# xuanvinh1997/llm-fp8

Measured on AMD Instinct MI355X. Metric: train tokens/sec + FP8 GEMM % of MFMA peak, Llama-3.2-3B seq512 b16, higher is better.
Workload: dtype fp8 (E4M3/E5M2 operands, fp32 accumulate, bf16 activations); 1 GPU; llama-3.2-3b (28 layers) full fine-tuning step, batch 16/GPU x seq 512, fp8_scenario=default (te_llama counterpart, lm_head FP8 under the outer recipe), random-init weights, synthetic tokens; route=fused, global_batch=16, seq_len=512, parallelism=single

## Files before the change

### llm_fp8_amd/csrc/mi_gemm.hip

```cpp
#include "mi_gemm_dev.h"
#include <algorithm>
#include <atomic>
#include <cstdlib>
#include <cstring>
#include <type_traits>

namespace mi {

template <int OUT>
__device__ __forceinline__ void store4(void* D, int64_t ldd, int64_t m, int64_t n0, v4f v) {
  if (OUT == 0) {
    uint2 p = make_uint2(pack_bf16x2(v[0], v[1]), pack_bf16x2(v[2], v[3]));
    *reinterpret_cast<uint2*>(reinterpret_cast<uint16_t*>(D) + m * ldd + n0) = p;
  } else {
    *reinterpret_cast<v4f*>(reinterpret_cast<float*>(D) + m * ldd + n0) = v;
  }
}

template <int FA, int FB, int OUT, bool MX>
__global__ __launch_bounds__(256) void gemm_generic(const uint8_t* __restrict__ A, const uint8_t* __restrict__ B,
                                                    void* __restrict__ D, const float* __restrict__ sa_inv,
                                                    const float* __restrict__ sb_inv,
                                                    const uint8_t* __restrict__ SA, const uint8_t* __restrict__ SB,
                                                    const uint16_t* __restrict__ bias, int M, int N, int K,
// ... 694 lines not shown
#pragma unroll
    for (int r = 0; r < nr; ++r)
#pragma unroll
      for (int st = 0; st < 4; ++st) epi_step(a_c, r0 + r, st, d_tile, zero, r == 0);
  };
  auto epilogue_block = [&](int ti, bool zero) __attribute__((always_inline)) {
    const int d_tile = tile_d_off(ti);
    epi_rows(c0_t{}, 0, 4, d_tile, ti & 1, zero);
    epi_rows(c1_t{}, 0, MA1, d_tile, ti & 1, zero);
  };
  auto mseg = [&](auto ni_c, auto nj_c, auto mf, auto a_c, auto nr_c, int r0, bool on, int d_tile, int bslot, bool zero)
                  __attribute__((always_inline)) {
    constexpr int NI = decltype(ni_c)::value, NJ = decltype(nj_c)::value, NM = NI * NJ;
    constexpr int SPR = kHybrid ? 3 : 4;
    constexpr int NR = decltype(nr_c)::value, NE = SPR * NR, MAXU = NR == 0 ? 0 : (NE + NM - 1) / NM;
    if (NR > 0 && on) epi_begin(bslot);
#pragma unroll
    for (int i = 0; i < NI; ++i)
#pragma unroll
      for (int j = 0; j < NJ; ++j) {
        mf(i, j);
        if (NR > 0) {
          const int k = i * NJ + j;
          if (on) {
#pragma unroll
            for (int u = 0; u < MAXU; ++u) {
              const int e = k * NE / NM + u;
              if (e < (k + 1) * NE / NM) epi_step(a_c, r0 + e / SPR, e % SPR, d_tile, zero, e < SPR, kHybrid ? e / SPR : 0);
            }
          }
          __builtin_amdgcn_sched_barrier(0);
        }
      }
  };

  constexpr bool kWoven = ABL == 14 || ABL == 16;
  auto lseg_store = [&](auto a_c, auto nr_c, int r0, bool on, int d_tile) __attribute__((always_inline)) {
    constexpr int NR = decltype(nr_c)::value;
    if (NR > 0 && kHybrid) {
      if (on) {
#pragma unroll
        for (int r = 0; r < NR; ++r) epi_step(a_c, r0 + r, 3, d_tile, false, false, r);
      }
      __builtin_amdgcn_sched_barrier(0);
    }
  };
  auto lseg_epi = [&](auto a_c, auto nr_c, int r0, bool on, int d_tile, int bslot, bool zero) __attribute__((always_inline)) {
    constexpr int NR = decltype(nr_c)::value;
    if (NR > 0 && !kWoven) {
      if (on) epi_rows(a_c, r0, NR, d_tile, bslot, zero);
      __builtin_amdgcn_sched_barrier(0);
    }
  };

  auto ktile = [&](auto mode_c, uint8_t* cur, uint8_t* oth, bool flag, int slot, int d_tile, int bslot) {
    constexpr int MODE = decltype(mode_c)::value;
    constexpr bool ZC = MODE == 1 && !MX;
    using nr01_t = std::integral_constant<int, (MODE == 1 ? MA1 / 2 : 0)>;
    using nr23_t = std::integral_constant<int, (MODE >= 3 ? 2 : 0)>;
    using wv01_t = std::integral_constant<int, (kWoven ? nr01_t::value : 0)>;
    using wv23_t = std::integral_constant<int, (kWoven ? nr23_t::value : 0)>;
    using ma1_t = std::integral_constant<int, MA1>;
    using nb1_t = std::integral_constant<int, NB1>;
    const int sa1 = oa_1 + keff(ti_1, kt_1) * BK, sb1 = ob_1 + keff(ti_1, kt_1) * BK;
    const int sa2 = oa_2 + keff(ti_2, kt_2) * BK, sb2 = ob_2 + keff(ti_2, kt_2) * BK;
    auto frag2 = [&](int lo, int hi, int off) __attribute__((always_inline)) -> v8i {
      const v4i l = *reinterpret_cast<const __attribute__((address_space(3))) v4i*>((size_t)(unsigned)(lo + off));
      const v4i h = *reinterpret_cast<const __attribute__((address_space(3))) v4i*>((size_t)(unsigned)(hi + off));
      return (v8i){l[0], l[1], l[2], l[3], h[0], h[1], h[2], h[3]};
    };
    auto frag = [&](int half_off, int, int g) __attribute__((always_inline)) -> v8i {
      if (half_off == kOffA0) return frag2(fa_lo, fa_hi, g * 2048);
      if (half_off == kOffB0) return frag2(fb_lo, fb_hi, g * 2048);
      if (half_off == kOffA1) return MA1 == 4 ? frag2(fa_lo, fa_hi, kHalfBytes + g * 2048) : frag2(fa1_lo, fa1_hi, g * 2048);
      return NB1 == 2 ? frag2(fb_lo, fb_hi, kHalfBytes + g * 2048) : frag2(fb1_lo, fb1_hi, g * 2048);
    };
    constexpr bool kE01 = !kWoven && nr01_t::value > 0, kE23 = !kWoven && nr23_t::value > 0;
    constexpr bool kH1 = kHybrid && MODE == 1, kH3 = kHybrid && MODE >= 3;
    using h2_t = std::integral_constant<int, 2>;
    using hm_t = std::integral_constant<int, MA1 / 2>;
    if (kE01 || kH1) {
      stage_scales(slot ^ 1, kt_1, ra_1, rb_1);
      stage_bias(ti_1 & 1, rb_1);
      stage_b1(sb1, oth);
      if (kH1) lseg_store(c0_t{}, h2_t{}, 2, flag, d_tile);
      else lseg_epi(c1_t{}, nr01_t{}, 0, flag, d_tile, bslot, MX);
    }
#pragma unroll
    for (int j = 0; j < 2; ++j) b0f[j] = frag(kOffB0, wc * 2, j);
#pragma unroll
    for (int i = 0; i < 4; ++i) af[i] = frag(kOffA0, wr * 4, i);
    if (MX && ABL != 5) {
#pragma unroll
      for (int j = 0; j < 2; ++j) asm volatile("ds_read_u8 %0, %1 offset:%2" : "=v"(b0s[j]) : "v"(sc_b), "n"(j * 16));
#pragma unroll
      for (int j = 0; j < NB1; ++j) asm volatile("ds_read_u8 %0, %1 offset:%2" : "=v"(b1s[j]) : "v"(sc_b), "n"(RB0 + j * 16));
      asm volatile("ds_read_b32 %0, %1" : "=v"(as_[0]) : "v"(sc_a));
      if (MA1 == 4) asm volatile("ds_read_b32 %0, %1" : "=v"(as1[0]) : "v"(sc_a1));
      else asm volatile("ds_read_u16 %0, %1" : "=v"(as1[0]) : "v"(sc_a1));
      if (ABL == 6) {
        asm volatile("" ::"v"(as_[0]), "v"(as1[0]));
        as_[0] = kUnitScale;
        as1[0] = kUnitScale;
#pragma unroll
        for (int j = 0; j < 2; ++j) {
          asm volatile("" ::"v"(b0s[j]), "v"(b1s[j]));
          b0s[j] = kUnitScale;
          b1s[j] = kUnitScale;
        }
      }
    }
    if (!(kE01 || kH1)) {
      stage_scales(slot ^ 1, kt_1, ra_1, rb_1);
      stage_bias(ti_1 & 1, rb_1);
      stage_b1(sb1, oth);
    }
    MI_WAIT_SYNC(MODE, flag, 0)
    stamp();
    mseg(c4_t{}, c2_t{}, [&](int i, int j) __attribute__((always_inline)) {
      if (ZC) mfma_ba_zero<FA, FB>(af[i], b0f[j], acc[0][i][0][j], b0s[j]);
      else acc[0][i][0][j] = mfma_sel(i, af[i], b0f[j], acc[0][i][0][j], as_, b0s[j]);
    }, c1_t{}, wv01_t{}, 0, flag, d_tile, bslot, MX);
    MI_PIN(4, 2, acc[0][i][0][j])
    MI_PHASE_END();
    stamp();
    if (kE01 || kH1) {
      stage_a1(sa1, oth);
      if (kH1) lseg_store(c1_t{}, hm_t{}, 0, flag, d_tile);
      else lseg_epi(c1_t{}, nr01_t{}, MA1 / 2, flag, d_tile, bslot, MX);
    }
#pragma unroll
    for (int j = 0; j < NB1; ++j) b1f[j] = frag(kOffB1, wc * NB1, j);
    if (!(kE01 || kH1)) stage_a1(sa1, oth);
    MI_WAIT_SYNC(MODE, flag, 1)
    stamp();
    mseg(c4_t{}, nb1_t{}, [&](int i, int j) __attribute__((always_inline)) {
      if (ZC) mfma_ba_zero<FA, FB>(af[i], b1f[j], acc[0][i][1][j], b1s[j]);
      else acc[0][i][1][j] = mfma_sel(i, af[i], b1f[j], acc[0][i][1][j], as_, b1s[j]);
    }, c1_t{}, wv01_t{}, MA1 / 2, flag, d_tile, bslot, MX);
    MI_PIN(4, NB1, acc[0][i][1][j])
    MI_PHASE_END();
    stamp();
    if (kE23 || kH1) {
      stage_a0(sa2, cur);
      if (kH1) lseg_store(c1_t{}, hm_t{}, MA1 / 2, flag, d_tile);
      else lseg_epi(c0_t{}, nr23_t{}, 0, true, d_tile, bslot, MX);
    }
#pragma unroll
    for (int i = 0; i < MA1; ++i) af[i] = frag(kOffA1, wr * MA1, i);
    if (!(kE23 || kH1)) stage_a0(sa2, cur);
    MI_WAIT_SYNC(MODE, flag, 2)
    stamp();
    mseg(ma1_t{}, nb1_t{}, [&](int i, int j) __attribute__((always_inline)) {
      if (ZC) mfma_ba_zero<FA, FB>(af[i], b1f[j], acc[1][i][1][j], b1s[j]);
      else acc[1][i][1][j] = mfma_sel(i, af[i], b1f[j], acc[1][i][1][j], as1, b1s[j]);
    }, c0_t{}, wv23_t{}, 0, true, d_tile, bslot, MX);
    MI_PIN(MA1, NB1, acc[1][i][1][j])
    MI_PHASE_END();
    stamp();
    stage_b0(sb2, cur);
    if (kH3) lseg_store(c0_t{}, h2_t{}, 0, true, d_tile);
    lseg_epi(c0_t{}, nr23_t{}, 2, true, d_tile, bslot, MX);
    MI_WAIT_SYNC(MODE, flag, 3)
    stamp();
    mseg(ma1_t{}, c2_t{}, [&](int i, int j) __attribute__((always_inline)) {
      if (ZC) mfma_ba_zero<FA, FB>(af[i], b0f[j], acc[1][i][0][j], b0s[j]);
      else acc[1][i][0][j] = mfma_sel(i, af[i], b0f[j], acc[1][i][0][j], as1, b0s[j]);
    }, c0_t{}, wv23_t{}, 2, true, d_tile, bslot, MX);
    frag_toggle();
    MI_PIN(MA1, 2, acc[1][i][0][j])
    MI_PHASE_END();
    stamp();
    ++s;
    advance(ti_1, kt_1, oa_1, ob_1, ra_1, rb_1, s + 1);
    advance(ti_2, kt_2, oa_2, ob_2, ra_2, rb_2, s + 2);
  };

  const rsrc_t rsW = __builtin_amdgcn_make_buffer_rsrc((void*)(SK ? (void*)sk_ws : (void*)A), 0, SK ? G * (8 * 32 * 1024) : 0, 0x00020000);
  auto partial_store = [&](int slot) {
    const int base = (slot * 8 + wave) * (32 * 1024);
#pragma unroll
    for (int a = 0; a < 2; ++a)
#pragma unroll
      for (int i = 0; i < (a == 0 ? 4 : MA1); ++i)
#pragma unroll
        for (int b = 0; b < 2; ++b)
#pragma unroll
          for (int j = 0; j < (b == 0 ? 2 : NB1); ++j) {
            const v4f v = acc[a][i][b][j];
            __builtin_amdgcn_raw_buffer_store_b128(__builtin_bit_cast(mi::v4u, v), rsW, lane * 16, base + (((a * 4 + i) * 2 + b) * 2 + j) * 1024, 16);
            asm volatile("s_nop 1" ::"v"(v) : "memory");
            acc[a][i][b][j] = (v4f){0.f, 0.f, 0.f, 0.f};
          }
    asm volatile("s_waitcnt vmcnt(0)" ::: "memory");
    __builtin_amdgcn_s_barrier();
    if (wave == 4 && lane == 0) __hip_atomic_store(sk_flags + slot, sk_epoch, __ATOMIC_RELEASE, __HIP_MEMORY_SCOPE_AGENT);
  };
  auto partial_add = [&](int slot) {
    if (lane == 0) {
      while (__hip_atomic_load(sk_flags + slot, __ATOMIC_ACQUIRE, __HIP_MEMORY_SCOPE_AGENT) != sk_epoch) __builtin_amdgcn_s_sleep(8);
    }
    __builtin_amdgcn_wave_barrier();
    const int base = (slot * 8 + wave) * (32 * 1024);
#pragma unroll
    for (int a = 0; a < 2; ++a)
#pragma unroll
      for (int i = 0; i < (a == 0 ? 4 : MA1); ++i)
#pragma unroll
        for (int b = 0; b < 2; ++b)
#pragma unroll
          for (int j = 0; j < (b == 0 ? 2 : NB1); ++j) {
            const mi::v4u w = __builtin_amdgcn_raw_buffer_load_b128(rsW, lane * 16, base + (((a * 4 + i) * 2 + b) * 2 + j) * 1024, 16);
            acc[a][i][b][j] += __builtin_bit_cast(v4f, w);
          }
  };

  unsigned long long dg_c0 = 0, dg_r0 = 0;
  if (ABL == 8) {
    dg_c0 = __builtin_amdgcn_s_memtime();
    dg_r0 = __builtin_amdgcn_s_memrealtime();
  }
  if constexpr (SK || !DEPI) {
    int kt = SK ? sk_k0 : 0, ti = 0;
    bool after = false;
    for (int pair = 0; pair < total / 2; ++pair) {
      ktile(c0_t{}, buf0, buf1, after, 0, 0, 0);
      ktile(c0_t{}, buf1, buf0, false, 1, 0, 0);
      after = false;
      kt += 2;
      if (kt == nk) {
        if (SK && ti == 0 && sk_k0 != 0) {
          partial_store(sk_v);
        } else {
          epilogue_block(ti, true);
          after = true;
        }
        kt = 0;
        ++ti;
      }
    }
    if (wr == 0) __builtin_amdgcn_s_barrier();
    asm volatile("s_waitcnt vmcnt(0)" ::: "memory");
    if (SK && kt != 0) {
      partial_add(sk_v + 1);
      epilogue_block(ti, false);
      asm volatile("s_waitcnt vmcnt(0)" ::: "memory");
    }
  } else {
    int d_prev = 0;
    using c4m_t = std::integral_constant<int, 4>;
    if (nk == 2) {
      for (int ti = 0; ti < my_tiles; ++ti) {
        const bool have_prev = ti > 0;
        ktile(c1_t{}, buf0, buf1, have_prev, 0, d_prev, (ti - 1) & 1);
        d_prev = tile_d_off(ti);
        ktile(c4m_t{}, buf1, buf0, have_prev, 1, d_prev, ti & 1);
      }
    } else {
      for (int ti = 0; ti < my_tiles; ++ti) {
        const bool have_prev = ti > 0;
        ktile(c1_t{}, buf0, buf1, have_prev, 0, d_prev, (ti - 1) & 1);
        ktile(c2_t{}, buf1, buf0, have_prev, 1, 0, 0);
        for (int pair = 2; pair < nk / 2; ++pair) {
          ktile(c0_t{}, buf0, buf1, false, 0, 0, 0);
          ktile(c0_t{}, buf1, buf0, false, 1, 0, 0);
        }
        d_prev = tile_d_off(ti);
        ktile(c0_t{}, buf0, buf1, false, 0, 0, 0);
        ktile(c3_t{}, buf1, buf0, true, 1, d_prev, ti & 1);
      }
    }
    if (wr == 0) __builtin_amdgcn_s_barrier();
    asm volatile("s_waitcnt vmcnt(0)" ::: "memory");
    if (my_tiles > 0) {
      if (kHybrid) {
        epi_step(c0_t{}, 2, 3, d_prev, false, false, 0);
        epi_step(c0_t{}, 3, 3, d_prev, false, false, 1);
      }
      epi_rows(c1_t{}, 0, MA1, d_prev, (my_tiles - 1) & 1, false);
    }
    if (ABL == 9) {
      if (blockIdx.x == 0 && (wave & 3) == 0) {
        asm volatile("s_waitcnt lgkmcnt(0)" ::: "memory");
        unsigned long long* dbg = (unsigned long long*)bias + (wave >> 2) * 1024;
        for (int i = lane; i < 1024; i += 64) dbg[i] = i < stamp_idx ? stamp_lds[i] : 0ull;
      }
    }
    if (ABL == 8) {
      const unsigned long long c1 = __builtin_amdgcn_s_memtime(), r1 = __builtin_amdgcn_s_memrealtime();
      if (tid == 0) {
        unsigned long long* dbg = (unsigned long long*)bias + (size_t)bid * 4;
        dbg[0] = c1 - dg_c0;
        dbg[1] = r1 - dg_r0;
        dbg[2] = (unsigned long long)total;
        dbg[3] = (unsigned long long)__builtin_amdgcn_s_getreg((20 << 0) | (0 << 6) | (3 << 11));
      }
    }
  }
#undef MI_WAIT_SYNC
#undef MI_PIN
}


static int pick_tile_cfg(int64_t M, int64_t N, int64_t K) {
  const double cold = 1.0 + 1150.0 / (double)(K > 0 ? K : 1);
  const double eff[4] = {1.0, 0.88 / cold, 0.92, 0.80 / cold};
  const int ncu = num_cus();
  int best = -1;
  double best_cost = 0;
  for (int c = 0; c < 4; ++c) {
    if (M % kTileBm[c] || N % kTileBn[c]) continue;
    const int64_t tiles = (M / kTileBm[c]) * (N / kTileBn[c]);
    const int64_t rounds = (tiles + ncu - 1) / ncu;
    const double cost = (double)rounds * kTileBm[c] * kTileBn[c] / eff[c];
    if (best < 0 || cost < best_cost * 0.98) {
      best = c;
      best_cost = cost;
    }
  }
  return best;
}

struct SkWorkspace {
  unsigned int* flags = nullptr;
  float* slots = nullptr;
  int nslots = 0;
};
static SkWorkspace g_sk_ws[32];
static std::atomic<unsigned int> g_sk_epoch{1};

static const SkWorkspace* sk_workspace() {
  int dev = 0;
  if (hipGetDevice(&dev) != hipSuccess || dev < 0 || dev >= 32) return nullptr;
  return g_sk_ws[dev].flags ? &g_sk_ws[dev] : nullptr;
}

static int sk_units(int64_t M, int64_t N, int64_t K) {
  if (M % 256 || N % 256 || K % 256) return 0;
  const SkWorkspace* ws = sk_workspace();
  const int ncu = num_cus();
  if (!ws || ws->nslots < ncu) return 0;
  const int64_t ntiles = (M / 256) * (N / 256), nk = K / BK;
  if (ntiles <= ncu || ntiles % ncu == 0) return 0;
  int64_t U = (ntiles * nk + ncu - 1) / ncu;
  U += U & 1;
  return U >= nk ? (int)U : 0;
}

enum ShapeClass { kAnyShape, kFastOk, kP8Ok, kP8Ok256 };
constexpr int kPick = -1;
constexpr int kCfgById = -2;
constexpr int kNoBuild = -1;

struct AlgoRow {
  int lo, hi;
  int family, build, sched, tile_cfg;
  bool one_tile_per_wg;
  bool lab;
  ShapeClass shape;
  bool mx_ok;
  BiasUse bias;
  bool e4m3_only;
};

constexpr AlgoRow kAlgos[] = {
    {1, 1,   kFamGeneric, 0,  0, kPick,    0, 0, kAnyShape, 1, kBiasAdded,   0},
    {2, 2,   kFam2Phase,  0,  0, kPick,    0, 0, kFastOk,   0, kBiasAdded,   0},
    {3, 3,   kFam8Phase,  0,  0, kPick,    0, 0, kFastOk,   0, kBiasAdded,   0},
    {4, 4,   kFamP8,      0,  0, kPick,    0, 0, kP8Ok,     1, kBiasAdded,   0},
    {5, 5,   kFamP8,      0,  0, kPick,    1, 0, kP8Ok,     1, kBiasAdded,   0},
    {6, 6,   kFamW4,      0,  0, 0,        1, 0, kP8Ok256,  0, kBiasRefused, 0},
    {7, 8,   kFamW4,      1,  0, 0,        1, 1, kP8Ok256,  0, kBiasRefused, 0},
    {9, 9,   kFamW4P,     0,  0, 0,        0, 0, kP8Ok256,  0, kBiasAdded,   0},
    {10, 12, kFamW4P,     1,  0, 0,        0, 1, kP8Ok256,  0, kBiasRefused, 1},
    {13, 14, kFam8Phase,  1,  0, kPick,    0, 1, kFastOk,   0, kBiasAdded,   0},
    {15, 15, kFamP8,      1,  0, kPick,    0, 1, kP8Ok,     0, kBiasUnused,  1},
    {16, 22, kFamP8,      3,  0, kPick,    0, 1, kP8Ok,     0, kBiasUnused,  1},
    {23, 23, kFamP8, kNoBuild, 0, kPick,   0, 1, kP8Ok,     0, kBiasUnused,  1},
    {24, 30, kFamP8,      11, 0, kPick,    0, 1, kP8Ok,     0, kBiasUnused,  1},
    {40, 43, kFamP8,      0,  0, kCfgById, 0, 0, kP8Ok,     1, kBiasAdded,   0},
    {44, 44, kFamStreamK, 0,  0, 0,        0, 0, kP8Ok,     1, kBiasAdded,   0},
    {45, 45, kFamP8,      0,  0, kPick,    0, 0, kP8Ok,     1, kBiasAdded,   0},
    {46, 46, kFamP8, kP8BlockEpilogue, 0, kPick, 0, 1, kP8Ok, 0, kBiasUnused, 1},
    {54, 56, kFamW4,      0,  1, 0,        1, 1, kP8Ok256,  0, kBiasUnused,  1},
    {62, 64, kFamW4,      0,  3, 0,        1, 1, kP8Ok256,  0, kBiasUnused,  1},
    {66, 68, kFamW4,      0,  4, 0,        1, 1, kP8Ok256,  0, kBiasUnused,  1},
    {50, 69, kFamW4, kNoBuild, 0, 0,       1, 1, kP8Ok256,  0, kBiasUnused,  1},
    {70, 73, kFamW4P,     4,  0, 0,        0, 1, kP8Ok256,  0, kBiasUnused,  1},
};

#ifdef MI_DIAG
constexpr bool kLabLibrary = true;
#else
constexpr bool kLabLibrary = false;
#endif

enum GemmEntry { kEntryFp8 = 0, kEntryMx, kEntryClock };
static const char* const kWho[] = {"mi_gemm_fp8", "mi_gemm_mxfp8", "mi_gemm_fp8_clock"};

static int plan_gemm(int entry, int64_t M, int64_t N, int64_t K, int64_t lda, int64_t ldb, int64_t ldd, int fa, int fb, int out,
                     bool has_bias, int algo, GemmPlan& p) {
  const bool mx = entry == kEntryMx, e4m3 = fa == 0 && fb == 0;
  auto find = [](int id) -> const AlgoRow* {
    for (const AlgoRow& r : kAlgos)
      if (id >= r.lo && id <= r.hi) return &r;
    return nullptr;
  };
  auto build_of = [](const AlgoRow& r, int id) { return r.build == kNoBuild || r.tile_cfg == kCfgById ? r.build : r.build + (id - r.lo); };
  auto mx_only = [](const AlgoRow& r, int build) { return r.family == kFamP8 && (build == 5 || build == 6); };
  p = GemmPlan{};
  if (mx) {
    MI_CHECK_ARG(K % 32 == 0, "mi_gemm_mxfp8: K must be a multiple of 32");
    const AlgoRow* r = find(algo);
    const bool listed = r && (r->mx_ok || mx_only(*r, build_of(*r, algo))) && (kLabLibrary || !r->lab);
    MI_CHECK_ARG(algo == 0 || listed, "mi_gemm_mxfp8: algo must be 0, 1, 4, 5%s or 40-45", kLabLibrary ? ", 18, 19" : "");
  }
  if (entry == kEntryClock) MI_CHECK_ARG(algo == 0 || algo == 4 || algo == 9, "mi_gemm_fp8_clock: algo must be 0, 4 or 9");
  if (M == 0 || N == 0) return MI_OK;

  const bool fast_ok = (M % BM == 0) && (N % BN == 0) && (K % BK == 0) && K > 0;
  const bool p8_ok = (M % 256 == 0 || M % 192 == 0) && (N % 256 == 0 || N % 192 == 0) && K > 0 && (K % (2 * BK) == 0) &&
                     out == 0 && M * lda < (1LL << 31) && N * ldb < (1LL << 31) && M * ldd * 2 < (1LL << 31);
  const bool p8_ok_256 = p8_ok && M % 256 == 0 && N % 256 == 0;
  const int ncu = num_cus();
  const int64_t tiles_256 = (M / 256) * (N / 256);
  if (algo == 47) {
    algo = (p8_ok_256 && K >= 512 && pick_tile_cfg(M, N, K) == 0 && (tiles_256 + ncu - 1) / ncu <= 64) ? 9 : 0;
  }
  if (algo == 0) algo = p8_ok ? 4 : ((fast_ok && !mx) ? 3 : 1);
  MI_CHECK_SHAPE(entry != kEntryClock || algo == 4 || algo == 9, "mi_gemm_fp8_clock: the shape does not run on a persistent kernel");
  const AlgoRow* r = find(algo);
  MI_CHECK_ARG(r == nullptr || !r->lab || kLabLibrary,
               "%s: algo %d is a timing / diagnostic build; it lives in the lab library (make -C llm_fp8_amd/csrc lab)", kWho[entry], algo);
  MI_CHECK_ARG(r != nullptr, "%s: unknown algo %d", kWho[entry], algo);
  const bool shape_ok[] = {true, fast_ok, p8_ok, p8_ok_256};
  static const char* const kNeeds[] = {"", "M,N % 256 == 0 and K % 128 == 0",
                                       "M,N % 256 (or 192) == 0, K % 256 == 0, bf16 output, operands < 2 GiB",
                                       "M,N,K % 256 == 0, bf16 output, operands < 2 GiB"};
  MI_CHECK_SHAPE(shape_ok[r->shape], "%s: algo %d needs %s", kWho[entry], algo, kNeeds[r->shape]);
  p.algo = algo;
  p.family = r->family;
  p.build = build_of(*r, algo);
  if (entry == kEntryClock) p.build = r->family == kFamP8 ? 8 : 2;
  const bool stamps = r->family == kFamP8    ? p.build == 8 || p.build == 9
                      : r->family == kFamW4P ? p.build == 2 || p.build == 7
                                             : (r->family == kFamW4 || r->family == kFam8Phase) && p.build == 2;
  MI_CHECK_ARG(!has_bias || stamps || r->bias != kBiasRefused,
               "mi_gemm: of the four-wave kernels only the persistent one (algo 9) takes a bias (got algo %d)", algo);
  p.sched = r->sched;
  p.mx = mx;
  p.tile_cfg = r->tile_cfg == kCfgById ? algo - r->lo : r->tile_cfg;
  p.tiles_m = (int)(M / 256);
  p.tiles_n = (int)(N / 256);
  p.one_tile_per_wg = r->one_tile_per_wg;
  p.bias_use = stamps ? kBiasIsStamps : (r->bias == kBiasAdded && has_bias) ? kBiasAdded : kBiasUnused;
  p.grid_x = (int)tiles_256;
  p.grid_y = 1;
  p.block = (r->family == kFamGeneric || r->family == kFamW4 || r->family == kFamW4P) ? 256 : 512;
  const int w4_number = r->family == kFamW4P ? 10 + p.build : 20 + (algo - 50);

  switch (r->family) {
    case kFamGeneric:
      p.grid_x = (int)((N + 63) / 64);
      p.grid_y = (int)((M + 63) / 64);
      break;
    case kFamStreamK:
      p.sk_units = sk_units(M, N, K);
      MI_CHECK_SHAPE(p.sk_units > 0, "mi_gemm: stream-K needs a registered workspace, 256-aligned M/N/K and more tiles than CUs (%lld x %lld x %lld)",
                     (long long)M, (long long)N, (long long)K);
      p.grid_x = (int)((tiles_256 * (K / BK) + p.sk_units - 1) / p.sk_units);
      break;
    case kFamP8: {
      const int cfg = p.tile_cfg == kPick ? pick_tile_cfg(M, N, K) : p.tile_cfg;
      MI_CHECK_SHAPE(cfg >= 0 && M % kTileBm[cfg] == 0 && N % kTileBn[cfg] == 0, "mi_gemm: no persistent tile shape divides %lld x %lld",
                     (long long)M, (long long)N);
      MI_CHECK_ARG(e4m3 || !r->e4m3_only, "mi_gemm: diagnostic algo %d is built for E4M3 x E4M3 only", algo);
      MI_CHECK_ARG(p.build != kNoBuild, "mi_gemm: unknown diagnostic algo %d", algo);
      MI_CHECK_SHAPE(p.build != 16 || K >= 512, "mi_gemm: algo %d needs K >= 512", algo);
      MI_CHECK_ARG(mx || !mx_only(*r, p.build), "mi_gemm: diagnostic algo %d reads MXFP8 block scales: call it through mi_gemm_mxfp8",
                   algo);
      p.tile_cfg = cfg;
      p.tiles_m = (int)(M / kTileBm[cfg]);
      p.tiles_n = (int)(N / kTileBn[cfg]);
      const int tiles = p.tiles_m * p.tiles_n;
      p.grid_x = (r->one_tile_per_wg || tiles < ncu) ? tiles : ncu;
#ifdef MI_DIAG
      if ((p.build == 3 || p.build == 8 || p.build == 9) && getenv("MI_GEMM_GRID"))
        p.grid_x = std::max(1, std::min(p.grid_x, atoi(getenv("MI_GEMM_GRID"))));
#endif
      break;
    }
    case kFamW4:
      MI_CHECK_ARG(e4m3 || !r->e4m3_only, "mi_gemm (w4): variant %d is a timing build of the lab library", w4_number);
      MI_CHECK_ARG(p.build != kNoBuild, "mi_gemm (w4): no such schedule variant %d", w4_number);
      break;
    case kFamW4P:
      p.grid_x = (int)(tiles_256 < ncu ? tiles_256 : ncu);
      MI_CHECK_SHAPE((tiles_256 + p.grid_x - 1) / p.grid_x <= 64 && K >= 512 && M / 256 < 16384 && N / 256 < 16384,
                     "mi_gemm (w4 persistent): needs K >= 512, at most 64 tiles per workgroup and fewer than 16384 tiles per dimension");
      MI_CHECK_ARG(e4m3 || p.build != 2, "mi_gemm (w4): the clock-stamp build is E4M3 x E4M3 only");
      MI_CHECK_ARG(e4m3 || !r->e4m3_only, "mi_gemm (w4): timing variant %d is built for E4M3 x E4M3 only", w4_number);
      break;
  }
  return MI_OK;
}


#ifdef MI_DIAG
#define MI_P8_BUILDS_E4M3(X)                                                                                               \
  X(1, false) X(3, false) X(4, false) X(5, true) X(6, true) X(7, false) X(8, false) X(9, false) X(11, false) X(12, false) \
  X(13, false) X(14, false) X(15, false) X(16, false) X(17, false) X(kP8BlockEpilogue, false)
#else
#define MI_P8_BUILDS_E4M3(X) X(8, false)
#endif

template <int FA, int FB, bool MX, bool BIAS, int ABL, bool DEPI = true, bool SK = false>
static void launch_p8_build(const GemmPlan& p, const GemmArgs& g) {
  const SkWorkspace* ws = SK ? sk_workspace() : nullptr;
  unsigned int epoch = SK ? g_sk_epoch.fetch_add(1) : 0u;
  if (SK && epoch == 0) epoch = g_sk_epoch.fetch_add(1);
  int last = p.sk_units;
#ifdef MI_DIAG
  if (ABL == 3 && getenv("MI_GEMM_STAGGER")) last = atoi(getenv("MI_GEMM_STAGGER"));
#endif
#define MI_P8_TILE(MA1, NB1)                                                                                                    \
  hipLaunchKernelGGL((gemm_256_p8<FA, FB, ABL, MX, BIAS, MA1, NB1, SK, DEPI>), dim3(p.grid_x), dim3(p.block), 0, g.st, g.A, g.B, \
                     (uint16_t*)g.D, g.sa_inv, g.sb_inv, (int)g.K, (int)g.lda, (int)g.ldb, (int)g.ldd, p.tiles_m, p.tiles_n,     \
                     (int)(g.M * g.lda), (int)(g.N * g.ldb), (int)(g.M * g.ldd * 2), g.SA, g.SB, (int)g.M, (int)g.N,             \
                     (const uint16_t*)g.bias, SK ? ws->slots : nullptr, SK ? ws->flags : nullptr, epoch, last)
  if constexpr (SK) {
    MI_P8_TILE(4, 2);
  } else {
    switch (p.tile_cfg) {
      case 0: MI_P8_TILE(4, 2); break;
      case 1: MI_P8_TILE(4, 1); break;
      case 2: MI_P8_TILE(2, 2); break;
      default: MI_P8_TILE(2, 1); break;
    }
  }
#undef MI_P8_TILE
}

template <int FA, int FB>
static int launch_p8(const GemmPlan& p, const GemmArgs& g) {
  if (p.build != 0 && (FA != 0 || FB != 0)) MI_NOT_COMPILED(p);
  switch (p.build) {
    case 0:
      with_pair(p.mx, p.bias_use == kBiasAdded, [&](auto mx, auto bias) {
        if (p.family == kFamStreamK) launch_p8_build<FA, FB, mx() != 0, bias() != 0, 0, true, true>(p, g);
        else launch_p8_build<FA, FB, mx() != 0, bias() != 0, 0>(p, g);
        return 0;
      });
      break;
#define MI_P8_BUILD(ABLv, MXv) \
  case ABLv: launch_p8_build<0, 0, MXv, false, (ABLv == kP8BlockEpilogue ? 0 : ABLv), ABLv != kP8BlockEpilogue>(p, g); break;
      MI_P8_BUILDS_E4M3(MI_P8_BUILD)
#undef MI_P8_BUILD
    default: MI_NOT_COMPILED(p);
  }
  MI_CHECK_LAUNCH(p.family == kFamStreamK ? "mi_gemm (stream-K) launch" : "mi_gemm (persistent) launch");
  return MI_OK;
}

template <int FA, int FB, int OUT>
static int launch_plain(const GemmPlan& p, const GemmArgs& g) {
  const dim3 grid(p.grid_x, p.grid_y), block(p.block);
  const uint16_t* bias = (const uint16_t*)g.bias;
#define MI_TILED(kernel)                                                                                                  \
  hipLaunchKernelGGL(kernel, grid, block, 0, g.st, g.A, g.B, g.D, g.sa_inv, g.sb_inv, bias, (int)g.M, (int)g.N, (int)g.K, \
                     g.lda, g.ldb, g.ldd, p.tiles_m, p.tiles_n)
#define MI_GENERIC(MXv)                                                                                                    \
  hipLaunchKernelGGL((gemm_generic<FA, FB, OUT, MXv>), grid, block, 0, g.st, g.A, g.B, g.D, g.sa_inv, g.sb_inv, g.SA, g.SB, \
                     bias, (int)g.M, (int)g.N, (int)g.K, g.lda, g.ldb, g.ldd)
  switch (p.family * 4 + p.build) {
    case kFamGeneric * 4: if (p.mx) MI_GENERIC(true); else MI_GENERIC(false); break;
    case kFam2Phase * 4: MI_TILED((gemm_256_2ph<FA, FB, OUT>)); break;
    case kFam8Phase * 4: MI_TILED((gemm_256_8ph<FA, FB, OUT>)); break;
#ifdef MI_DIAG
    case kFam8Phase * 4 + 1: MI_TILED((gemm_256_8ph<FA, FB, OUT, 1>)); break;
    case kFam8Phase * 4 + 2: MI_TILED((gemm_256_8ph<FA, FB, OUT, 2>)); break;
#endif
    default: MI_NOT_COMPILED(p);
  }
#undef MI_GENERIC
#undef MI_TILED
  MI_CHECK_LAUNCH("mi_gemm launch");
  return MI_OK;
}

static int launch_gemm(const GemmPlan& p, const GemmArgs& g) {
  if (p.family == kFamW4 || p.family == kFamW4P) return launch_w4(p, g);
  return with_pair(g.fa, g.fb, [&](auto fa, auto fb) -> int {
    constexpr int FA = fa(), FB = fb();
    if (p.family == kFamP8 || p.family == kFamStreamK) return launch_p8<FA, FB>(p, g);
    return g.out == 0 ? launch_plain<FA, FB, 0>(p, g) : launch_plain<FA, FB, 1>(p, g);
  });
}

static int check_common(const char* who, const void* A, const void* B, const void* D, int64_t M, int64_t N, int64_t K,
                        int64_t lda, int64_t ldb, int64_t ldd, int fa, int fb, int out) {
  MI_CHECK_ARG(A && B && D, "%s: null operand", who);
  MI_CHECK_ARG(M >= 0 && N >= 0 && K >= 0, "%s: negative shape", who);
  MI_CHECK_ARG(M % 8 == 0 && N % 8 == 0 && K % 16 == 0, "%s: M,N must be multiples of 8 and K of 16 (got %lld,%lld,%lld)",
               who, (long long)M, (long long)N, (long long)K);
  MI_CHECK_ARG(M < (1LL << 31) && N < (1LL << 31) && K < (1LL << 31), "%s: shape too large", who);
  MI_CHECK_ARG(lda >= K && ldb >= K && ldd >= N && lda % 16 == 0 && ldb % 16 == 0 && ldd % 4 == 0,
               "%s: bad leading dimensions", who);
  MI_CHECK_ARG(((uintptr_t)A % 16) == 0 && ((uintptr_t)B % 16) == 0 && ((uintptr_t)D % 16) == 0,
               "%s: operands must be 16-byte aligned", who);
  MI_CHECK_ARG((fa == 0 || fa == 1) && (fb == 0 || fb == 1) && (out == 0 || out == 1), "%s: bad fmt/out_dtype", who);
  return MI_OK;
}

static int run_gemm(int entry, const GemmArgs& g, int algo) {
  int rc = check_common(kWho[entry], g.A, g.B, g.D, g.M, g.N, g.K, g.lda, g.ldb, g.ldd, g.fa, g.fb, g.out);
  if (rc != MI_OK) return rc;
  const bool scales = entry == kEntryMx ? g.SA && g.SB : g.sa_inv && g.sb_inv;
  MI_CHECK_ARG(scales && (entry != kEntryClock || g.bias), "%s: null %spointer", kWho[entry], entry == kEntryClock ? "" : "scale ");
  GemmPlan p;
  rc = plan_gemm(entry, g.M, g.N, g.K, g.lda, g.ldb, g.ldd, g.fa, g.fb, g.out, entry != kEntryClock && g.bias != nullptr, algo, p);
  if (rc != MI_OK || p.family == kFamNone) return rc;
  return launch_gemm(p, g);
}

}

extern "C" int mi_gemm_fp8(const void* A, const void* B, void* D, const float* sa_inv, const float* sb_inv,
                           const void* bias_bf16, int64_t M, int64_t N, int64_t K, int64_t lda, int64_t ldb,
                           int64_t ldd, int fmt_a, int fmt_b, int out_dtype, int algo, void* stream) {
  return mi::run_gemm(mi::kEntryFp8, {(const uint8_t*)A, (const uint8_t*)B, D, sa_inv, sb_inv, nullptr, nullptr, bias_bf16, M, N, K,
                                      lda, ldb, ldd, fmt_a, fmt_b, out_dtype, (hipStream_t)stream}, algo);
}

extern "C" int mi_gemm_fp8_clock(const void* A, const void* B, void* D, const float* sa_inv, const float* sb_inv, int64_t M,
                                 int64_t N, int64_t K, int64_t lda, int64_t ldb, int64_t ldd, int algo, unsigned long long* stamps,
                                 void* stream) {
  return mi::run_gemm(mi::kEntryClock, {(const uint8_t*)A, (const uint8_t*)B, D, sa_inv, sb_inv, nullptr, nullptr, stamps, M, N, K,
                                        lda, ldb, ldd, 0, 0, 0, (hipStream_t)stream}, algo);
}

extern "C" int mi_gemm_mxfp8(const void* A, const void* SA, const void* B, const void* SB, void* D,
                             const void* bias_bf16, int64_t M, int64_t N, int64_t K, int fmt_a, int fmt_b,
                             int out_dtype, int algo, void* stream) {
  return mi::run_gemm(mi::kEntryMx, {(const uint8_t*)A, (const uint8_t*)B, D, nullptr, nullptr, (const uint8_t*)SA, (const uint8_t*)SB,
                                     bias_bf16, M, N, K, K, K, N, fmt_a, fmt_b, out_dtype, (hipStream_t)stream}, algo);
}

#ifdef MI_DIAG
extern "C" int mi_gemm_plan_diag(int entry, int64_t M, int64_t N, int64_t K, int64_t lda, int64_t ldb, int64_t ldd, int fmt_a,
                                 int fmt_b, int out_dtype, int has_bias, int algo, mi_gemm_plan* out) {
  MI_CHECK_ARG(entry >= 0 && entry <= 2 && out != nullptr, "mi_gemm_plan_diag: bad entry or null plan");
  const void* aligned = (const void*)16;
  int rc = mi::check_common(mi::kWho[entry], aligned, aligned, aligned, M, N, K, lda, ldb, ldd, fmt_a, fmt_b, out_dtype);
  return rc != MI_OK ? rc : mi::plan_gemm(entry, M, N, K, lda, ldb, ldd, fmt_a, fmt_b, out_dtype, has_bias != 0, algo, *out);
}
#endif

extern "C" int64_t mi_gemm_workspace_bytes(void) { return 4096 + (int64_t)mi::num_cus() * (8 * 32 * 1024); }

extern "C" int mi_gemm_set_workspace(void* workspace, int64_t bytes) {
  int dev = 0;
  if (hipGetDevice(&dev) != hipSuccess || dev < 0 || dev >= 32) {
    mi::set_error("mi_gemm_set_workspace: no current device");
    return MI_ERR_HIP;
  }
  if (workspace == nullptr) {
    mi::g_sk_ws[dev] = mi::SkWorkspace();
    return MI_OK;
  }
  MI_CHECK_ARG(((uintptr_t)workspace & 255) == 0, "mi_gemm_set_workspace: pointer must be 256-byte aligned");
  MI_CHECK_ARG(bytes >= 4096 + 8 * 32 * 1024, "mi_gemm_set_workspace: %lld bytes is too small", (long long)bytes);
  mi::SkWorkspace w;
  w.flags = (unsigned int*)workspace;
  w.slots = (float*)((char*)workspace + 4096);
  w.nslots = (int)((bytes - 4096) / (8 * 32 * 1024));
  if (w.nslots > 1024) w.nslots = 1024;
  mi::g_sk_ws[dev] = w;
  return MI_OK;
}
```

### llm_fp8_amd/csrc/mi_gemm_w4.hip

```cpp
#include "mi_gemm_dev.h"
#include <type_traits>
#include <utility>

namespace mi {

template <class F, int... I>
__device__ __forceinline__ void static_for_impl(F&& f, std::integer_sequence<int, I...>) {
  (f(std::integral_constant<int, I>{}), ...);
}
template <int N, class F>
__device__ __forceinline__ void static_for(F&& f) {
  static_for_impl(f, std::make_integer_sequence<int, N>{});
}

template <int FA, int FB>
__device__ __forceinline__ void mfma_acc(const v8i& a, const v8i& b, v4f& acc, int unit) {
  asm volatile("v_mfma_scale_f32_16x16x128_f8f6f4 %0, %1, %2, %0, %3, %3 op_sel_hi:[0,0,0] cbsz:%4 blgp:%5"
               : "+a"(acc)
               : "v"(b), "v"(a), "v"(unit), "n"(FB), "n"(FA));
}

namespace w4 {
constexpr int sched_lag(int S) { return (S == 3 || S == 4) ? 2 : 1; }
constexpr int sched_kb(int S) { return 0; }
constexpr int sched_dm(int S, int p) { return S == 1 ? 1 + 4 * p : S == 3 ? 2 + 4 * p : 1 + p; }
constexpr int sched_rd(int S, int n) { return S == 3 ? 1 + 2 * n : 4 + n; }
}

template <int FA, int FB, int ABL, int S = 0>
__global__ __launch_bounds__(256, 1) void gemm_w4(const uint8_t* __restrict__ A, const uint8_t* __restrict__ B,
                                                  uint16_t* __restrict__ D, const float* __restrict__ sa_inv,
                                                  const float* __restrict__ sb_inv, int K, int lda, int ldb, int ldd,
                                                  int tiles_m, int tiles_n, int a_bytes, int b_bytes, int d_bytes,
                                                  unsigned long long* __restrict__ dbg) {
  constexpr int LAG = w4::sched_lag(S);
  __shared__ __attribute__((aligned(16))) uint8_t lds[kLdsBytes];
  const int tid = threadIdx.x, lane = tid & 63;
  const int wave = __builtin_amdgcn_readfirstlane(tid >> 6);
  const int wr = wave >> 1, wc = wave & 1;
  int tm, tn;
  tile_of_block(blockIdx.x, gridDim.x, tiles_m, tiles_n, tm, tn);
  const rsrc_t rsA = __builtin_amdgcn_make_buffer_rsrc((void*)A, 0, a_bytes, 0x00020000);
  const rsrc_t rsB = __builtin_amdgcn_make_buffer_rsrc((void*)B, 0, b_bytes, 0x00020000);
  const int oa = tm * 256 * lda, ob = tn * 256 * ldb;
  const int nk = K / BK, last = nk - 1;

  int a_v, b_v;
  {
    const int lr = lane >> 3, lc = lane & 7;
    const int chunk = (lc ^ swz_f(lr)) * 16;
    const int row = (wave >> 1) * 128 + (wave & 1) * 32 + lr;
    a_v = row * lda + chunk;
    b_v = row * ldb + chunk;
  }
  uint8_t* const buf0 = lds;
  uint8_t* const buf1 = lds + kBufBytes;
  auto dma = [&](rsrc_t rs, uint8_t* dst, int voff, int soff) __attribute__((always_inline)) {
    __builtin_amdgcn_raw_ptr_buffer_load_lds(rs, LDS_PTR(dst), 16, voff, soff, 0, 0);
  };
  auto stage_a = [&](int h, int kt, uint8_t* buf, int p) __attribute__((always_inline)) {
    dma(rsA, buf + (h ? kOffA1 : kOffA0) + (wave * 4 + p) * 1024, a_v, oa + min(kt, last) * BK + (h * 64 + p * 8) * lda);
  };
  auto stage_b = [&](int h, int kt, uint8_t* buf, int p) __attribute__((always_inline)) {
    dma(rsB, buf + (h ? kOffB1 : kOffB0) + (wave * 4 + p) * 1024, b_v, ob + min(kt, last) * BK + (h * 64 + p * 8) * ldb);
  };

  int fa_lo[2], fa_hi[2], fb_lo[2], fb_hi[2];
  {
    const int r = lane & 15, q = lane >> 4;
    const int frow = (r >> 3) * 1024 + (r & 7) * 128;
    const int flo = frow + ((q ^ swz_f(r)) << 4), fhi = frow + (((4 + q) ^ swz_f(r)) << 4);
    const int l0 = (int)(size_t)LDS_PTR(lds);
#pragma unroll
    for (int b = 0; b < 2; ++b) {
      fa_lo[b] = l0 + b * kBufBytes + kOffA0 + wr * 4 * 2048 + flo;
      fa_hi[b] = l0 + b * kBufBytes + kOffA0 + wr * 4 * 2048 + fhi;
      fb_lo[b] = l0 + b * kBufBytes + kOffB0 + wc * 4 * 2048 + flo;
      fb_hi[b] = l0 + b * kBufBytes + kOffB0 + wc * 4 * 2048 + fhi;
    }
  }
  typedef const __attribute__((address_space(3))) v4i* lds_v4i_p;
  auto read_part = [&](v8i (&dst)[4], int lo, int hi, int half, int n) __attribute__((always_inline)) {
    const int f = n >> 1;
    const v4i v = *reinterpret_cast<lds_v4i_p>((size_t)(unsigned)(((n & 1) ? hi : lo) + half * kHalfBytes + f * 2048));
    if (n & 1) dst[f].hi = v;
    else dst[f].lo = v;
  };

  v4f acc[2][2][4][4];
#pragma unroll
  for (int a = 0; a < 2; ++a)
#pragma unroll
    for (int b = 0; b < 2; ++b)
#pragma unroll
      for (int i = 0; i < 4; ++i)
#pragma unroll
        for (int j = 0; j < 4; ++j) acc[a][b][i][j] = (v4f){0.f, 0.f, 0.f, 0.f};
  v8i aA[4], aB[4], b0[2][4], b1[4];
  int unit = kUnitScale;
  asm volatile("" : "+v"(unit));

  constexpr int kVm = LAG == 1 ? 24 : 20;
  auto phase = [&](const v8i (&af)[4], const v8i (&bf)[4], v4f (&c)[4][4], auto stage, auto read) __attribute__((always_inline)) {
    __builtin_amdgcn_sched_barrier(0);
#pragma unroll
    for (int k = 0; k < 16; ++k) {
      const int i = k >> 2, j = k & 3;
      mfma_acc<FA, FB>(af[i], bf[j], c[i][j], unit);
      if (k == w4::sched_kb(S)) {
        __builtin_amdgcn_sched_barrier(0);
        if (LAG == 1) asm volatile("s_waitcnt vmcnt(24) lgkmcnt(0)" ::: "memory");
        else asm volatile("s_waitcnt vmcnt(20) lgkmcnt(8)" ::: "memory");
        __builtin_amdgcn_s_barrier();
      }
#pragma unroll
      for (int p = 0; p < 4; ++p)
        if (k == w4::sched_dm(S, p)) stage(p);
#pragma unroll
      for (int n = 0; n < 8; ++n)
        if (k == w4::sched_rd(S, n)) read(n);
      __builtin_amdgcn_sched_barrier(0);
    }
  };

  auto ktile = [&](auto par_c, int t) __attribute__((always_inline)) {
    constexpr int par = decltype(par_c)::value;
    uint8_t* const cur = par ? buf1 : buf0;
    uint8_t* const oth = par ? buf0 : buf1;
    if (LAG == 1) {
      phase(aA, b0[par], acc[0][0], [&](int p) __attribute__((always_inline)) { stage_b(0, t + 2, cur, p); },
            [&](int n) __attribute__((always_inline)) { read_part(b1, fb_lo[par], fb_hi[par], 1, n); });
      phase(aA, b1, acc[0][1], [&](int p) __attribute__((always_inline)) { stage_b(1, t + 2, cur, p); },
            [&](int n) __attribute__((always_inline)) { read_part(aB, fa_lo[par], fa_hi[par], 1, n); });
      phase(aB, b1, acc[1][1], [&](int p) __attribute__((always_inline)) { stage_a(1, t + 2, cur, p); },
            [&](int n) __attribute__((always_inline)) { read_part(aA, fa_lo[par ^ 1], fa_hi[par ^ 1], 0, n); });
      phase(aB, b0[par], acc[1][0], [&](int p) __attribute__((always_inline)) { stage_a(0, t + 3, oth, p); },
            [&](int n) __attribute__((always_inline)) { read_part(b0[par ^ 1], fb_lo[par ^ 1], fb_hi[par ^ 1], 0, n); });
    } else {
      phase(aA, b0[par], acc[0][0], [&](int p) __attribute__((always_inline)) { stage_a(0, t + 2, cur, p); },
            [&](int n) __attribute__((always_inline)) { read_part(b1, fb_lo[par], fb_hi[par], 1, n); });
      phase(aA, b1, acc[0][1], [&](int p) __attribute__((always_inline)) { stage_b(0, t + 2, cur, p); },
            [&](int n) __attribute__((always_inline)) { read_part(aB, fa_lo[par], fa_hi[par], 1, n); });
      phase(aB, b1, acc[1][1], [&](int p) __attribute__((always_inline)) { stage_b(1, t + 2, cur, p); },
            [&](int n) __attribute__((always_inline)) { read_part(aA, fa_lo[par ^ 1], fa_hi[par ^ 1], 0, n); });
      phase(aB, b0[par], acc[1][0], [&](int p) __attribute__((always_inline)) { stage_a(1, t + 2, cur, p); },
            [&](int n) __attribute__((always_inline)) { read_part(b0[par ^ 1], fb_lo[par ^ 1], fb_hi[par ^ 1], 0, n); });
    }
  };

  auto stage4a = [&](int h, int kt, uint8_t* buf) __attribute__((always_inline)) {
#pragma unroll
    for (int p = 0; p < 4; ++p) stage_a(h, kt, buf, p);
  };
  auto stage4b = [&](int h, int kt, uint8_t* buf) __attribute__((always_inline)) {
#pragma unroll
    for (int p = 0; p < 4; ++p) stage_b(h, kt, buf, p);
  };
  stage4a(0, 0, buf0);
  stage4b(0, 0, buf0);
  stage4b(1, 0, buf0);
  stage4a(1, 0, buf0);
  stage4a(0, 1, buf1);
  stage4b(0, 1, buf1);
  if (LAG == 1) {
    stage4b(1, 1, buf1);
    asm volatile("s_waitcnt vmcnt(24)" ::: "memory");
    __builtin_amdgcn_s_barrier();
    stage4a(1, 1, buf1);
#pragma unroll
    for (int n = 0; n < 8; ++n) read_part(aA, fa_lo[0], fa_hi[0], 0, n);
    asm volatile("s_waitcnt vmcnt(24) lgkmcnt(0)" ::: "memory");
    __builtin_amdgcn_s_barrier();
    stage4a(0, 2, buf0);
  } else {
    asm volatile("s_waitcnt vmcnt(20)" ::: "memory");
    __builtin_amdgcn_s_barrier();
    stage4b(1, 1, buf1);
#pragma unroll
    for (int n = 0; n < 8; ++n) read_part(aA, fa_lo[0], fa_hi[0], 0, n);
    asm volatile("s_waitcnt vmcnt(20)" ::: "memory");
    __builtin_amdgcn_s_barrier();
    stage4a(1, 1, buf1);
  }
#pragma unroll
  for (int n = 0; n < 8; ++n) read_part(b0[0], fb_lo[0], fb_hi[0], 0, n);
  __builtin_amdgcn_sched_barrier(0);

  unsigned long long c0 = 0, r0 = 0;
  if (ABL == 2) {
    c0 = __builtin_amdgcn_s_memtime();
    r0 = __builtin_amdgcn_s_memrealtime();
  }
  using par0_t = std::integral_constant<int, 0>;
  using par1_t = std::integral_constant<int, 1>;
  for (int t = 0; t < nk; t += 2) {
    ktile(par0_t{}, t);
    ktile(par1_t{}, t + 1);
  }
  if (ABL == 2) {
    const unsigned long long c1 = __builtin_amdgcn_s_memtime(), r1 = __builtin_amdgcn_s_memrealtime();
    if (tid == 0) {
      unsigned long long* o = dbg + (size_t)blockIdx.x * 4;
      o[0] = c1 - c0;
      o[1] = r1 - r0;
      o[2] = (unsigned long long)nk;
      o[3] = (unsigned long long)__builtin_amdgcn_s_getreg((20 << 0) | (0 << 6) | (3 << 11));
    }
  }
  asm volatile("s_waitcnt vmcnt(0) lgkmcnt(0)" ::: "memory");

  const float alpha = (*sa_inv) * (*sb_inv);
  const int fr = lane & 15, fq = lane >> 4;
#pragma unroll
  for (int a = 0; a < 2; ++a)
#pragma unroll
    for (int i = 0; i < 4; ++i)
#pragma unroll
      for (int b = 0; b < 2; ++b)
#pragma unroll
        for (int j = 0; j < 4; ++j) {
          const int64_t m = (int64_t)tm * 256 + wr * 128 + a * 64 + i * 16 + fr;
          const int64_t n = (int64_t)tn * 256 + wc * 128 + b * 64 + j * 16 + fq * 4;
          const v4f v = acc[a][b][i][j] * alpha;
          if (ABL != 0) {
            asm volatile("" ::"v"(v[0]), "v"(v[1]), "v"(v[2]), "v"(v[3]));
          } else {
            const uint2 pk = make_uint2(pack_bf16x2(v[0], v[1]), pack_bf16x2(v[2], v[3]));
            *reinterpret_cast<uint2*>(D + m * ldd + n) = pk;
          }
        }
}

namespace w4 {
constexpr int kPark = 5;
constexpr int conv_start(int r) { return r < 8 ? 19 + 8 * r : 80 + 5 * (r - 8); }
constexpr int store_slot(int e) { return 24 + 4 * e; }
constexpr int kFrameSlots = store_slot(31) + 4;
constexpr int stores_in_phase(int gp) {
  int n = 0;
  for (int e = 0; e < 32; ++e)
    if (store_slot(e) / 16 == gp) ++n;
  return n;
}
constexpr int wait_x(int G) {
  int n = 0;
  for (int q = G - 5; q < G; ++q)
    if (q >= 0) n += stores_in_phase(q);
  return n;
}
enum { MID = -1, LAST = 0, FIRST = 4, SECOND = 8, THIRD = 12 };
constexpr bool schedule_ok() {
  for (int r = 0; r < 16; ++r) {
    const int q = r / 4, i = r % 4;
    if (conv_start(r) < 16 + 16 * q) return false;
    if (conv_start(r) + 3 >= 64 + 16 * q + 4 * i + 3) return false;
    if (store_slot(2 * r) < conv_start(r) + 5) return false;
    if (r + kPark < 16 && conv_start(r + kPark) + 1 <= store_slot(2 * r + 1) + 3) return false;
  }
  return kFrameSlots <= 160;
}
static_assert(schedule_ok(), "epilogue schedule violates a deadline");
}

template <int FA, int FB>
__device__ __forceinline__ void mfma_acc_zero(const v8i& a, const v8i& b, v4f& acc, int unit) {
  asm volatile("v_mfma_scale_f32_16x16x128_f8f6f4 %0, %1, %2, 0, %3, %3 op_sel_hi:[0,0,0] cbsz:%4 blgp:%5"
               : "+a"(acc)
               : "v"(b), "v"(a), "v"(unit), "n"(FB), "n"(FA));
}

struct W4Single {
  const uint8_t* A;
  const uint8_t* B;
  uint16_t* D;
  const float* sa_inv;
  const float* sb_inv;
  const uint16_t* bias;
  unsigned long long* dbg;
  int K, lda, ldb, ldd, tiles_m, tiles_n, a_bytes, b_bytes, d_bytes, n_cols;
};

template <int FA, int FB, int ABL, int MODE>
__global__ __launch_bounds__(256, 1) void gemm_w4p(const std::conditional_t<MODE == 2, GroupArgs, W4Single> ka) {
  constexpr bool GROUPED = MODE == 2, BIAS = MODE == 1;
  constexpr int S = 3;
  static_assert(w4::sched_lag(S) == 2, "the cursor logic below assumes every stage of step s goes to step s + 2");
  static_assert(!(GROUPED && ABL != 0), "the grouped form has no timing builds");
  __shared__ __attribute__((aligned(16))) uint8_t lds[kLdsBytes + (ABL == 7 ? 8192 : 0)];
  int stamp_idx = 0;
  const int tid = threadIdx.x, lane = tid & 63;
  const int wave = __builtin_amdgcn_readfirstlane(tid >> 6);
  const int wr = wave >> 1, wc = wave & 1;
  const int G = gridDim.x, bid = blockIdx.x;

  int my_tiles = 0, tab = 0;
  float alpha_of[kMaxGroup] = {1.f, 1.f, 1.f, 1.f};
  if constexpr (GROUPED) {
    const int q8 = G >> 3, r8 = G & 7, xcd = bid & 7;
    const int v = (xcd < r8 ? xcd * (q8 + 1) : r8 * (q8 + 1) + (xcd - r8) * q8) + (bid >> 3);
    int my_cnt[kMaxGroup];
#pragma unroll
    for (int q = 0; q < kMaxGroup; ++q) {
      my_cnt[q] = q < ka.n ? (int)ka.cnt[q][v] : 0;
      my_tiles += my_cnt[q];
      float a = 1.0f;
      if (q < ka.n) a = (*ka.p[q].sa_inv) * (*ka.p[q].sb_inv);
      alpha_of[q] = __builtin_bit_cast(float, __builtin_amdgcn_readfirstlane(__builtin_bit_cast(int, a)));
    }
    int my_id = 0, my_p = 0, ti = 0;
#pragma unroll
    for (int q = 0; q < kMaxGroup; ++q) {
      if (q < ka.n) {
        const unsigned c4 = reinterpret_cast<const unsigned*>(ka.cnt[q])[lane];
        for (int j = 0; j < my_cnt[q]; ++j, ++ti) {
          int rank = 0;
#pragma unroll
          for (int k = 0; k < 4; ++k) {
            const bool f = (int)((c4 >> (8 * k)) & 255u) > j && (4 * lane + k) < v;
            rank += __builtin_popcountll(__builtin_amdgcn_ballot_w64(f));
          }
          if (lane == ti) {
            my_id = (int)ka.R[q][j] + rank;
            my_p = q;
          }
        }
      }
    }
    int tmn = ka.p[0].tiles_m, tnn = ka.p[0].tiles_n;
#pragma unroll
    for (int q = 1; q < kMaxGroup; ++q) {
      const bool is = my_p == q;
      tmn = is ? ka.p[q].tiles_m : tmn;
      tnn = is ? ka.p[q].tiles_n : tnn;
    }
    int tm, tn;
    tile_of_flat(my_id, max(tmn, 1), max(tnn, 1), tm, tn);
    tab = tm | (tn << 14) | (my_p << 28);
  } else {
    const int ntiles = ka.tiles_m * ka.tiles_n;
    my_tiles = (ntiles - bid + G - 1) / G;
    int tm, tn;
    tile_of_block(bid + min(lane, max(my_tiles - 1, 0)) * G, ntiles, ka.tiles_m, ka.tiles_n, tm, tn);
    tab = tm | (tn << 14);
    alpha_of[0] = (*ka.sa_inv) * (*ka.sb_inv);
  }
  auto tile_of = [&](int ti, int& p, int& ra, int& rb) __attribute__((always_inline)) {
    const int t = __builtin_amdgcn_readlane(tab, ti);
    p = (t >> 28) & 3;
    ra = (t & 0x3FFF) * 256;
    rb = ((t >> 14) & 0x3FFF) * 256;
  };

  uint8_t* const buf0 = lds;
  uint8_t* const buf1 = lds + kBufBytes;
  auto dma = [&](rsrc_t rs, uint8_t* dst_base, int voff, int soff, auto p_c) __attribute__((always_inline)) {
    constexpr int IMM = decltype(p_c)::value * 1024;
    __builtin_amdgcn_raw_ptr_buffer_load_lds(rs, LDS_PTR(dst_base), 16, voff, soff - IMM, IMM, 0);
  };
  struct cursor_t {
    int oa, ob, kb, ti, kt, nk, lda, ldb, a_v, b_v, step;
    rsrc_t rsA, rsB;
  };
  auto enter_tile = [&](cursor_t& c, int ti) __attribute__((always_inline)) {
    int p, ra, rb;
    tile_of(ti, p, ra, rb);
    if constexpr (GROUPED) {
      const GroupProblem& P = ka.p[p];
      c.nk = P.nk;
      c.lda = P.lda;
      c.ldb = P.ldb;
      c.rsA = __builtin_amdgcn_make_buffer_rsrc((void*)P.A, 0, (int)((unsigned)P.a_bytes + 4096u), 0x00020000);
      c.rsB = __builtin_amdgcn_make_buffer_rsrc((void*)P.B, 0, (int)((unsigned)P.b_bytes + 4096u), 0x00020000);
      int ln;
      asm volatile("v_mov_b32 %0, %1" : "=v"(ln) : "v"(lane));
      const int lr = ln >> 3, chunk = ((ln & 7) ^ swz_f(lr)) * 16;
      const int row = (wave >> 1) * 128 + (wave & 1) * 32 + lr;
      c.a_v = row * P.lda + chunk;
      c.b_v = row * P.ldb + chunk;
    }
    c.oa = ra * c.lda;
    c.ob = rb * c.ldb;
  };
  int total = 0;
  auto advance = [&](cursor_t& c) __attribute__((always_inline)) {
    if constexpr (GROUPED) {
      const bool wrap = c.kt + 1 == c.nk;
      if (wrap && c.ti + 1 < my_tiles) {
        c.ti += 1;
        c.kt = 0;
        c.kb = 0;
        enter_tile(c, c.ti);
      } else {
        const int inc = wrap ? 0 : 1;
        c.kt += inc;
        c.kb += inc * BK;
      }
    } else {
      const int more = (c.step + 1 < total) ? 1 : 0;
      c.step += more;
      const int kt1 = c.kt + more;
      const int wrap = (kt1 == c.nk) ? 1 : 0;
      c.kt = wrap ? 0 : kt1;
      c.kb = wrap ? 0 : c.kb + more * BK;
      c.ti += wrap;
      enter_tile(c, c.ti);
    }
  };
  auto stage_a = [&](int h, const cursor_t& c, uint8_t* buf, auto p_c) __attribute__((always_inline)) {
    constexpr int p = decltype(p_c)::value;
    dma(c.rsA, buf + (h ? kOffA1 : kOffA0) + wave * 4096, c.a_v, c.oa + c.kb + (h * 64 + p * 8) * c.lda, p_c);
  };
  auto stage_b = [&](int h, const cursor_t& c, uint8_t* buf, auto p_c) __attribute__((always_inline)) {
    constexpr int p = decltype(p_c)::value;
    dma(c.rsB, buf + (h ? kOffB1 : kOffB0) + wave * 4096, c.b_v, c.ob + c.kb + (h * 64 + p * 8) * c.ldb, p_c);
  };

  int fa_lo[2], fa_hi[2], fb_lo[2], fb_hi[2];
  {
    const int r = lane & 15, q = lane >> 4;
    const int frow = (r >> 3) * 1024 + (r & 7) * 128;
    const int flo = frow + ((q ^ swz_f(r)) << 4), fhi = frow + (((4 + q) ^ swz_f(r)) << 4);
    const int l0 = (int)(size_t)LDS_PTR(lds);
#pragma unroll
    for (int b = 0; b < 2; ++b) {
      fa_lo[b] = l0 + b * kBufBytes + kOffA0 + wr * 4 * 2048 + flo;
      fa_hi[b] = l0 + b * kBufBytes + kOffA0 + wr * 4 * 2048 + fhi;
      fb_lo[b] = l0 + b * kBufBytes + kOffB0 + wc * 4 * 2048 + flo;
      fb_hi[b] = l0 + b * kBufBytes + kOffB0 + wc * 4 * 2048 + fhi;
    }
  }
  typedef const __attribute__((address_space(3))) v4i* lds_v4i_p;
  auto read_part = [&](v8i (&dst)[4], int lo, int hi, int half, int n) __attribute__((always_inline)) {
    const int f = n >> 1;
    const v4i v = *reinterpret_cast<lds_v4i_p>((size_t)(unsigned)(((n & 1) ? hi : lo) + half * kHalfBytes + f * 2048));
    if (n & 1) dst[f].hi = v;
    else dst[f].lo = v;
  };

  v4f acc[2][2][4][4];
#pragma unroll
  for (int a = 0; a < 2; ++a)
#pragma unroll
    for (int b = 0; b < 2; ++b)
#pragma unroll
      for (int i = 0; i < 4; ++i)
#pragma unroll
        for (int j = 0; j < 4; ++j) acc[a][b][i][j] = (v4f){0.f, 0.f, 0.f, 0.f};
  v8i aA[4], aB[4], b0[2][4], b1[4];
  int unit = kUnitScale;
  asm volatile("" : "+v"(unit));

  struct epi_t {
    rsrc_t rs;
    int d_off, ldd, d_voff;
    float alpha;
  };
  auto epi_of = [&](int ti, bool real) __attribute__((always_inline)) -> epi_t {
    int p, ra, rb;
    tile_of(ti, p, ra, rb);
    epi_t e;
    uint16_t* Dp;
    int d_bytes;
    if constexpr (GROUPED) {
      const GroupProblem& P = ka.p[p];
      Dp = P.D;
      d_bytes = P.d_bytes;
      e.ldd = P.ldd;
      e.alpha = p == 0 ? alpha_of[0] : p == 1 ? alpha_of[1] : p == 2 ? alpha_of[2] : alpha_of[3];
    } else {
      Dp = ka.D;
      d_bytes = ka.d_bytes;
      e.ldd = ka.ldd;
      e.alpha = alpha_of[0];
    }
    e.rs = __builtin_amdgcn_make_buffer_rsrc((void*)Dp, 0, real ? d_bytes : 0, 0x00020000);
    e.d_off = (ra * e.ldd + rb) * 2;
    int ln;
    asm volatile("v_mov_b32 %0, %1" : "=v"(ln) : "v"(lane));
    const int fr = ln & 15, fq = ln >> 4;
    const int ecol = (fq & 1) * 16 + (fq >> 1) * 8;
    e.d_voff = ((wr * 128 + (fr & 7)) * e.ldd + wc * 128 + (fr >> 3) * 32 + ecol) * 2;
    return e;
  };
  v4i park[w4::kPark][2];
#pragma unroll
  for (int i = 0; i < w4::kPark; ++i) park[i][0] = park[i][1] = (v4i){0, 0, 0, 0};
  typedef unsigned int v2u_ __attribute__((ext_vector_type(2)));
  v2u_ bias_w[2][4];
#pragma unroll
  for (int b = 0; b < 2; ++b)
#pragma unroll
    for (int j = 0; j < 4; ++j) bias_w[b][j] = (v2u_){0u, 0u};
  u32 px = 0, py = 0;
  auto conv_chunk = [&](auto r_c, auto sub_c, const epi_t& e) __attribute__((always_inline)) {
    constexpr int r = decltype(r_c)::value, sub = decltype(sub_c)::value;
    constexpr int q = r >> 2, a = q >> 1, b = (q == 1 || q == 2) ? 1 : 0, i = r & 3;
    v4i& e0 = park[r % w4::kPark][0];
    v4i& e1 = park[r % w4::kPark][1];
    if constexpr (sub < 4) {
      asm volatile("" : "+a"(acc[a][b][i][sub]));
      const v4f t = acc[a][b][i][sub];
      float m0 = t[0] * e.alpha, m1 = t[1] * e.alpha, m2 = t[2] * e.alpha, m3 = t[3] * e.alpha;
      asm volatile("" : "+v"(m0), "+v"(m1), "+v"(m2), "+v"(m3));
      v4f v = {m0, m1, m2, m3};
      if constexpr (BIAS) {
        v[0] += __uint_as_float(bias_w[b][sub].x << 16);
        v[1] += __uint_as_float(bias_w[b][sub].x & 0xFFFF0000u);
        v[2] += __uint_as_float(bias_w[b][sub].y << 16);
        v[3] += __uint_as_float(bias_w[b][sub].y & 0xFFFF0000u);
      }
      const u32 x = pack_bf16x2(v[0], v[1]), y = pack_bf16x2(v[2], v[3]);
      if constexpr ((sub & 1) == 0) {
        px = x;
        py = y;
      } else {
        const auto sx = __builtin_amdgcn_permlane16_swap(px, x, false, false);
        const auto sy = __builtin_amdgcn_permlane16_swap(py, y, false, false);
        const v4i rr = {(int)sx[0], (int)sy[0], (int)sx[1], (int)sy[1]};
        if constexpr (sub == 1) e0 = rr;
        else e1 = rr;
      }
    } else {
#pragma unroll
      for (int k = 0; k < 4; ++k) {
        const int keep = e1[k];
        e1[k] = __builtin_amdgcn_update_dpp(e1[k], e0[k], 0x128, 0xF, 0x3, false);
        e0[k] = __builtin_amdgcn_update_dpp(e0[k], keep, 0x128, 0xF, 0xC, false);
      }
    }
  };
  auto store_event = [&](auto e_c, auto w_c, const epi_t& e) __attribute__((always_inline)) {
    constexpr int ev = decltype(e_c)::value, r = ev >> 1, half = ev & 1, w = decltype(w_c)::value;
    constexpr int q = r >> 2, a = q >> 1, b = (q == 1 || q == 2) ? 1 : 0, i = r & 3;
    const int rowoff = e.d_off + ((a * 64 + i * 16 + half * 8) * e.ldd + b * 64) * 2;
    const v4i data = park[r % w4::kPark][half];
    if (ABL == 1) {
      asm volatile("" ::"v"(data));
    } else {
      constexpr int kAux = ABL == 4 ? 0 : ABL == 5 ? 2 : ABL == 6 ? 18 : 16;
      if (wave == w) {
        __builtin_amdgcn_raw_buffer_store_b128((mi::v4u)data, e.rs, e.d_voff, rowoff, kAux);
        asm volatile("s_nop 1" ::"v"(data) : "memory");
      }
    }
  };
  auto epi_slot = [&](auto g_c, const epi_t& e) __attribute__((always_inline)) {
    constexpr int g = decltype(g_c)::value;
    if constexpr (ABL != 3) {
      static_for<16>([&](auto r_c) __attribute__((always_inline)) {
        constexpr int r = decltype(r_c)::value, cs = w4::conv_start(r);
        if constexpr (g >= cs && g < cs + 5) conv_chunk(r_c, std::integral_constant<int, g - cs>{}, e);
      });
      if constexpr (g >= w4::store_slot(0) && g < w4::kFrameSlots)
        store_event(std::integral_constant<int, (g - w4::store_slot(0)) / 4>{}, std::integral_constant<int, (g - w4::store_slot(0)) % 4>{}, e);
    }
  };
  rsrc_t rsBias = __builtin_amdgcn_make_buffer_rsrc((void*)lds, 0, 0, 0x00020000);
  if constexpr (BIAS) rsBias = __builtin_amdgcn_make_buffer_rsrc((void*)ka.bias, 0, ka.n_cols * 2, 0x00020000);
  auto load_bias = [&](int rb) __attribute__((always_inline)) {
    if constexpr (BIAS) {
      const int voff = (wc * 128 + (lane >> 4) * 4) * 2;
#pragma unroll
      for (int b = 0; b < 2; ++b)
#pragma unroll
        for (int j = 0; j < 4; ++j)
          bias_w[b][j] = __builtin_bit_cast(v2u_, __builtin_amdgcn_raw_buffer_load_b64(rsBias, voff, rb * 2 + (b * 64 + j * 16) * 2, 0));
    }
  };

  cursor_t c2;
  auto phase = [&](auto mode_c, auto p_c, const v8i (&af)[4], const v8i (&bf)[4], v4f (&c)[4][4], auto stage, auto read,
                   const epi_t& e, int rb_cur) __attribute__((always_inline)) {
    constexpr int MODE_ = decltype(mode_c)::value, P = decltype(p_c)::value;
    constexpr bool ZC = MODE_ == w4::FIRST;
    constexpr bool NOST = ABL == 1 || ABL == 3;
    constexpr int G_ = MODE_ + P;
    constexpr int XB = (BIAS && MODE_ != w4::MID && G_ >= 9 && G_ <= 13) ? 8 : 0;
    constexpr int X = ((NOST || MODE_ == w4::MID) ? 0 : w4::wait_x(G_)) + XB;
    static_assert(20 + X <= 63, "vmcnt is a 6-bit counter");
    __builtin_amdgcn_sched_barrier(0);
    static_for<16>([&](auto k_c) __attribute__((always_inline)) {
      constexpr int k = decltype(k_c)::value, i = k >> 2, j = k & 3;
      if constexpr (ZC) mfma_acc_zero<FA, FB>(af[i], bf[j], c[i][j], unit);
      else mfma_acc<FA, FB>(af[i], bf[j], c[i][j], unit);
      if constexpr (k == w4::sched_kb(S)) {
        __builtin_amdgcn_sched_barrier(0);
        asm volatile("s_waitcnt vmcnt(%0) lgkmcnt(8)" ::"n"(20 + X) : "memory");
        __builtin_amdgcn_s_barrier();
        if constexpr (BIAS && MODE_ == w4::SECOND && P == 0) load_bias(rb_cur);
      }
      static_for<4>([&](auto p_c) __attribute__((always_inline)) {
        if constexpr (k == w4::sched_dm(S, decltype(p_c)::value)) stage(p_c);
      });
#pragma unroll
      for (int n = 0; n < 8; ++n)
        if (k == w4::sched_rd(S, n)) read(n);
      if constexpr (MODE_ != w4::MID && MODE_ != w4::THIRD) epi_slot(std::integral_constant<int, 16 * (MODE_ + P) + k>{}, e);
      __builtin_amdgcn_sched_barrier(0);
    });
  };
  using p0_t = std::integral_constant<int, 0>;
  using p1_t = std::integral_constant<int, 1>;
  using p2_t = std::integral_constant<int, 2>;
  using p3_t = std::integral_constant<int, 3>;
  auto ktile = [&](auto mode_c, auto par_c, const epi_t& e, int rb_cur, auto simple_c) __attribute__((always_inline)) {
    constexpr int par = decltype(par_c)::value;
    constexpr bool SIMPLE = decltype(simple_c)::value;
    uint8_t* const cur = par ? buf1 : buf0;
    if (ABL == 7) {
      if (bid == 0 && wave == 0 && stamp_idx < 1024) {
        const unsigned long long t = __builtin_amdgcn_s_memtime();
        if (lane == 0) reinterpret_cast<unsigned long long*>(lds + kLdsBytes)[stamp_idx] = t;
      }
      ++stamp_idx;
    }
    phase(mode_c, p0_t{}, aA, b0[par], acc[0][0], [&](auto p) __attribute__((always_inline)) { stage_a(0, c2, cur, p); },
          [&](int n) __attribute__((always_inline)) { read_part(b1, fb_lo[par], fb_hi[par], 1, n); }, e, rb_cur);
    phase(mode_c, p1_t{}, aA, b1, acc[0][1], [&](auto p) __attribute__((always_inline)) { stage_b(0, c2, cur, p); },
          [&](int n) __attribute__((always_inline)) { read_part(aB, fa_lo[par], fa_hi[par], 1, n); }, e, rb_cur);
    phase(mode_c, p2_t{}, aB, b1, acc[1][1], [&](auto p) __attribute__((always_inline)) { stage_b(1, c2, cur, p); },
          [&](int n) __attribute__((always_inline)) { read_part(aA, fa_lo[par ^ 1], fa_hi[par ^ 1], 0, n); }, e, rb_cur);
    phase(mode_c, p3_t{}, aB, b0[par], acc[1][0], [&](auto p) __attribute__((always_inline)) { stage_a(1, c2, cur, p); },
          [&](int n) __attribute__((always_inline)) { read_part(b0[par ^ 1], fb_lo[par ^ 1], fb_hi[par ^ 1], 0, n); }, e, rb_cur);
    if constexpr (SIMPLE) {
      c2.step += 1;
      c2.kt += 1;
      c2.kb += BK;
    } else {
      advance(c2);
    }
  };

  if (my_tiles <= 0) return;
  c2.ti = 0; c2.kt = 0; c2.kb = 0; c2.step = 0;
  if constexpr (!GROUPED) {
    c2.nk = ka.K / BK;
    c2.lda = ka.lda;
    c2.ldb = ka.ldb;
    c2.rsA = __builtin_amdgcn_make_buffer_rsrc((void*)ka.A, 0, (int)((unsigned)ka.a_bytes + 4096u), 0x00020000);
    c2.rsB = __builtin_amdgcn_make_buffer_rsrc((void*)ka.B, 0, (int)((unsigned)ka.b_bytes + 4096u), 0x00020000);
    const int lr = lane >> 3, chunk = ((lane & 7) ^ swz_f(lr)) * 16;
    const int row = (wave >> 1) * 128 + (wave & 1) * 32 + lr;
    c2.a_v = row * ka.lda + chunk;
    c2.b_v = row * ka.ldb + chunk;
    total = my_tiles * c2.nk;
  }
  enter_tile(c2, 0);
  auto stage4a = [&](int h, uint8_t* buf) __attribute__((always_inline)) {
    static_for<4>([&](auto p_c) __attribute__((always_inline)) { stage_a(h, c2, buf, p_c); });
  };
  auto stage4b = [&](int h, uint8_t* buf) __attribute__((always_inline)) {
    static_for<4>([&](auto p_c) __attribute__((always_inline)) { stage_b(h, c2, buf, p_c); });
  };
  stage4a(0, buf0);
  stage4b(0, buf0);
  stage4b(1, buf0);
  stage4a(1, buf0);
  advance(c2);
  stage4a(0, buf1);
  stage4b(0, buf1);
  asm volatile("s_waitcnt vmcnt(20)" ::: "memory");
  __builtin_amdgcn_s_barrier();
  stage4b(1, buf1);
#pragma unroll
  for (int n = 0; n < 8; ++n) read_part(aA, fa_lo[0], fa_hi[0], 0, n);
  asm volatile("s_waitcnt vmcnt(20)" ::: "memory");
  __builtin_amdgcn_s_barrier();
  stage4a(1, buf1);
#pragma unroll
  for (int n = 0; n < 8; ++n) read_part(b0[0], fb_lo[0], fb_hi[0], 0, n);
  advance(c2);
  __builtin_amdgcn_sched_barrier(0);

  unsigned long long ck0 = 0, rt0 = 0;
  if (ABL == 2) {
    ck0 = __builtin_amdgcn_s_memtime();
    rt0 = __builtin_amdgcn_s_memrealtime();
  }
  using par0_t = std::integral_constant<int, 0>;
  using par1_t = std::integral_constant<int, 1>;
  using mid_t = std::integral_constant<int, w4::MID>;
  using first_t = std::integral_constant<int, w4::FIRST>;
  using second_t = std::integral_constant<int, w4::SECOND>;
  using third_t = std::integral_constant<int, w4::THIRD>;
  using last_t = std::integral_constant<int, w4::LAST>;
  epi_t ep_prev = epi_of(0, false);
  int steps_done = 0;
  for (int ti = 0; ti < my_tiles; ++ti) {
    const epi_t ep_cur = epi_of(ti, true);
    int p_, ra_, rb_cur;
    tile_of(ti, p_, ra_, rb_cur);
    int nk_t;
    if constexpr (GROUPED) nk_t = ka.p[p_].nk;
    else nk_t = ka.K / BK;
    using full_t = std::false_type;
    using simple_t = std::true_type;
    ktile(first_t{}, par0_t{}, ep_prev, rb_cur, full_t{});
    ktile(second_t{}, par1_t{}, ep_prev, rb_cur, full_t{});
    ktile(third_t{}, par0_t{}, ep_cur, rb_cur, full_t{});
    const int npair = nk_t / 2;
    for (int pair = 2; pair < npair - 1; ++pair) {
      ktile(mid_t{}, par1_t{}, ep_cur, rb_cur, simple_t{});
      ktile(mid_t{}, par0_t{}, ep_cur, rb_cur, simple_t{});
    }
    if (npair > 2) {
      ktile(mid_t{}, par1_t{}, ep_cur, rb_cur, full_t{});
      ktile(mid_t{}, par0_t{}, ep_cur, rb_cur, full_t{});
    }
    ktile(last_t{}, par1_t{}, ep_cur, rb_cur, full_t{});
    ep_prev = ep_cur;
    steps_done += nk_t;
  }
  if (ABL == 2) {
    const unsigned long long ck1 = __builtin_amdgcn_s_memtime(), rt1 = __builtin_amdgcn_s_memrealtime();
    if (tid == 0) {
      if constexpr (!GROUPED) {
        unsigned long long* o = ka.dbg + (size_t)bid * 4;
        o[0] = ck1 - ck0;
        o[1] = rt1 - rt0;
        o[2] = (unsigned long long)steps_done;
        o[3] = (unsigned long long)__builtin_amdgcn_s_getreg((20 << 0) | (0 << 6) | (3 << 11));
      }
    }
  }
  if (ABL == 7) {
    const unsigned long long t_end = __builtin_amdgcn_s_memtime();
    if constexpr (!GROUPED) {
      if (bid == 0 && wave == 0) {
        asm volatile("s_waitcnt lgkmcnt(0)" ::: "memory");
        for (int i = lane; i < 1024; i += 64)
          ka.dbg[i] = i < stamp_idx ? reinterpret_cast<unsigned long long*>(lds + kLdsBytes)[i] : (i == stamp_idx ? t_end : 0ull);
      }
    }
  }
  asm volatile("s_waitcnt vmcnt(0) lgkmcnt(0)\n\ts_nop 7\n\ts_nop 7" ::: "memory");
  static_for<w4::kFrameSlots - 64>([&](auto g_c) __attribute__((always_inline)) {
    epi_slot(std::integral_constant<int, 64 + decltype(g_c)::value>{}, ep_prev);
    __builtin_amdgcn_sched_barrier(0);
  });
}

#ifdef MI_DIAG
#define MI_W4_BUILDS(X) X(0, 0) X(1, 0) X(2, 0) X(0, 1) X(1, 1) X(2, 1) X(0, 3) X(1, 3) X(2, 3) X(0, 4) X(1, 4) X(2, 4)
#define MI_W4P_BUILDS_E4M3(X) X(1) X(2) X(3) X(4) X(5) X(6) X(7)
#else
#define MI_W4_BUILDS(X) X(0, 0)
#define MI_W4P_BUILDS_E4M3(X) X(2)
#endif

int launch_w4(const GemmPlan& p, const GemmArgs& g) {
  return with_pair(g.fa, g.fb, [&](auto fa, auto fb) -> int {
    constexpr int FA = fa(), FB = fb();
    const dim3 grid(p.grid_x), block(p.block);
    unsigned long long* dbg = p.bias_use == kBiasIsStamps ? (unsigned long long*)g.bias : nullptr;
    uint16_t* D = (uint16_t*)g.D;
    if (p.family == kFamW4) {
#define MI_W4(ABLv, Sv)                                                                                                   \
  case ABLv * 8 + Sv:                                                                                                     \
    hipLaunchKernelGGL((gemm_w4<(Sv ? 0 : FA), (Sv ? 0 : FB), ABLv, Sv>), grid, block, 0, g.st, g.A, g.B, D, g.sa_inv,     \
                       g.sb_inv, (int)g.K, (int)g.lda, (int)g.ldb, (int)g.ldd, p.tiles_m, p.tiles_n, (int)(g.M * g.lda),  \
                       (int)(g.N * g.ldb), (int)(g.M * g.ldd * 2), dbg);                                                  \
    break;
      if (p.sched != 0 && (FA != 0 || FB != 0)) MI_NOT_COMPILED(p);
      switch (p.build * 8 + p.sched) {
        MI_W4_BUILDS(MI_W4)
        default: MI_NOT_COMPILED(p);
      }
#undef MI_W4
    } else {
      W4Single ws;
      ws.A = g.A; ws.B = g.B; ws.D = D; ws.sa_inv = g.sa_inv; ws.sb_inv = g.sb_inv; ws.dbg = dbg;
      ws.bias = p.bias_use == kBiasAdded ? (const uint16_t*)g.bias : nullptr;
      ws.K = (int)g.K; ws.lda = (int)g.lda; ws.ldb = (int)g.ldb; ws.ldd = (int)g.ldd; ws.tiles_m = p.tiles_m; ws.tiles_n = p.tiles_n;
      ws.a_bytes = (int)(g.M * g.lda); ws.b_bytes = (int)(g.N * g.ldb); ws.d_bytes = (int)(g.M * g.ldd * 2); ws.n_cols = (int)g.N;
      if (p.build != 0 && (FA != 0 || FB != 0)) MI_NOT_COMPILED(p);
#define MI_W4P(ABLv) case ABLv: hipLaunchKernelGGL((gemm_w4p<0, 0, ABLv, 0>), grid, block, 0, g.st, ws); break;
      switch (p.build) {
        case 0:
          if (ws.bias) hipLaunchKernelGGL((gemm_w4p<FA, FB, 0, 1>), grid, block, 0, g.st, ws);
          else hipLaunchKernelGGL((gemm_w4p<FA, FB, 0, 0>), grid, block, 0, g.st, ws);
          break;
        MI_W4P_BUILDS_E4M3(MI_W4P)
        default: MI_NOT_COMPILED(p);
      }
#undef MI_W4P
    }
    MI_CHECK_LAUNCH("mi_gemm (w4) launch");
    return MI_OK;
  });
}

int launch_w4_grouped(const GroupArgs& ga, int fa, int fb, int grid, hipStream_t st) {
  for (int q = 0; q < ga.n; ++q)
    if (ga.p[q].nk < 4 || (ga.p[q].nk & 1)) {
      set_error("mi_gemm_fp8_grouped (four-wave kernel): every problem needs K >= 512 and K %% 256 == 0");
      return MI_ERR_SHAPE;
    }
  with_pair(fa, fb, [&](auto a, auto b) {
    hipLaunchKernelGGL((gemm_w4p<a(), b(), 0, 2>), dim3(grid), dim3(256), 0, st, ga);
    return 0;
  });
  MI_CHECK_LAUNCH("mi_gemm_fp8_grouped (four-wave) launch");
  return MI_OK;
}

}
```

### llm_fp8_amd/pytorch/module.py

```python
from __future__ import annotations

import io
import os
from typing import List, Optional, Sequence, Tuple

import torch
import torch.nn.functional as F

from ..common.recipe import DelayedScaling, Float8BlockScaling, Float8CurrentScaling, Format, MXFP8BlockScaling, Recipe, fmt_codes
from . import ops
from .fp8 import FP8GlobalStateManager, ModuleMeta

__all__ = ["Linear", "LayerNormLinear", "LayerNormMLP", "LayerNorm", "RMSNorm"]


def _as_bf16_2d(t: torch.Tensor) -> torch.Tensor:
    t2 = t.reshape(-1, t.shape[-1])
    if t2.dtype != torch.bfloat16:
        t2 = t2.to(torch.bfloat16)
    return t2.contiguous()


class DyHandoff:
    __slots__ = ("scale", "amax", "fmt", "want_y", "want_t", "fp8", "ptr", "mx", "act_ref")
# ... 236 lines not shown

    def __init__(self, fmt_f: int, fmt_b: int):
        self.fmt_f, self.fmt_b = fmt_f, fmt_b

    def quantize(self, x2, g: int, want_t: bool, norm=None):
        if norm is None:
            q = ops.mxfp8_quantize(x2, self.fmt_f, rowwise=True, colwise=want_t)
        else:
            q = ops.mxfp8_norm_quantize(x2, norm[0], norm[1], self.fmt_f, rowwise=True, colwise=want_t)
        return q[:2], q[2:]

    def swiglu(self, h, g: int, want_t: bool, bias):
        assert bias is None
        q = ops.mxfp8_swiglu_quantize(h, self.fmt_f, rowwise=True, colwise=want_t)
        return q[:2], q[2:]

    def quantize_grad(self, g2, g: int, want_y: bool, want_t: bool, colsum: bool = False):
        q = ops.mxfp8_quantize(g2, self.fmt_b, rowwise=want_y, colwise=want_t, want_colsum=colsum)
        return q[:2], q[2:4], q[4] if colsum else None

    def dswiglu(self, h, dact, g: int, want_y: bool, want_t: bool, colsum: bool, bias):
        assert bias is None
        q = ops.mxfp8_dswiglu_quantize(h, dact, self.fmt_b, rowwise=want_y, colwise=want_t, want_colsum=colsum)
        return q[:2], q[2:4], q[4]

    def offer(self, handoff: DyHandoff, g: int, want_y: bool, want_t: bool) -> None:
        handoff.offer(None, None, self.fmt_b, want_y, want_t, mx=True)

    def taken(self, fp8, g: int):
        return fp8[:2], fp8[2:], None

    def operands(self, a, b):
        return a + b

    def gemm(self, a, b, bias):
        return ops.gemm_mxfp8(a[0], a[1], b[0], b[1], self.fmt_f, self.fmt_f, bias=bias)

    def unflat(self, flat):
        return flat[:2], flat[2:]

    def quantize_weights(self, weights, ns, N: int, K: int, dev, g: int, want_t: bool):
        fmt = self.fmt_f
        ws_ = [(w if w.dtype == torch.bfloat16 else w.to(torch.bfloat16)).contiguous() for w in weights]
        if len(ws_) == 1:
            return ops.mxfp8_quantize(ws_[0], fmt, rowwise=True, colwise=want_t)
        if any(n % 32 for n in ns):
            return ops.mxfp8_quantize(torch.cat(ws_, 0), fmt, rowwise=True, colwise=want_t)
        w8 = torch.empty((N, K), dtype=torch.uint8, device=dev)
        sc = torch.empty((K // 32, N), dtype=torch.uint8, device=dev)
        wt8 = torch.empty((K, N), dtype=torch.uint8, device=dev) if want_t else None
        sct = torch.empty((N // 32, K), dtype=torch.uint8, device=dev) if want_t else None
        r = 0
        for w, n in zip(ws_, ns):
            ops.mxfp8_quantize(w, fmt, rowwise=True, colwise=want_t,
                               out=(w8[r:r + n], sc[:, r:r + n], wt8[:, r:r + n] if want_t else None,
                                    sct[r // 32:(r + n) // 32] if want_t else None))
            r += n
        return w8, sc, wt8, sct

    def new_sink(self, weights, ns, N: int, K: int, dev, g: int):
        return MXWeightSink(weights, ns, N, K, dev) if N % 32 == 0 and K % 32 == 0 and all(n % 32 == 0 for n in ns) else None

    def refresh(self, dp, sink) -> None:
        dp.refresh_mx_operand(sink, self.fmt_f)

    def sink_flat(self, sink, g: int):
        return sink.w8, sink.sc, sink.wt8, sink.sct


class _BlockQ(_MXQ):
    __slots__ = ("recipe",)
    cache_key, sink_key = "blk", "blksink"
    no_sink = ("Float8BlockScaling keeps no optimiser-filled FP8 weight copies, which row-sharded weights (distributed.ShardedFP8DP, "
               "--sharding_mode fsdp_fp8) depend on: use --sharding_mode replicated (GradArenaDP) with this recipe")

    def __init__(self, recipe: Float8BlockScaling, fmt_f: int, fmt_b: int):
        super().__init__(fmt_f, fmt_b)
        self.recipe = recipe

    def quantize(self, x2, g: int, want_t: bool, norm=None):
        r = self.recipe
        dim, eps = r.x_block_scaling_dim, r.fp8_quant_fwd_inp.amax_epsilon
        if norm is None:
            q = ops.blockfp8_quantize(x2, self.fmt_f, dim, rowwise=True, colwise=want_t, amax_epsilon=eps)
        else:
            q = ops.blockfp8_norm_quantize(x2, norm[0], norm[1], self.fmt_f, dim, rowwise=True, colwise=want_t, amax_epsilon=eps)
        return q[:2], q[2:]

    def swiglu(self, h, g: int, want_t: bool, bias):
        assert bias is None
        r = self.recipe
        q = ops.blockfp8_swiglu_quantize(h, self.fmt_f, r.x_block_scaling_dim, rowwise=True, colwise=want_t,
                                         amax_epsilon=r.fp8_quant_fwd_inp.amax_epsilon)
        return q[:2], q[2:]

    def quantize_grad(self, g2, g: int, want_y: bool, want_t: bool, colsum: bool = False):
        r = self.recipe
        q = ops.blockfp8_quantize(g2, self.fmt_b, r.grad_block_scaling_dim, rowwise=want_y, colwise=want_t, want_colsum=colsum,
                                  amax_epsilon=r.fp8_quant_bwd_grad.amax_epsilon)
        return q[:2], q[2:4], q[4] if colsum else None

    def dswiglu(self, h, dact, g: int, want_y: bool, want_t: bool, colsum: bool, bias):
        assert bias is None
        r = self.recipe
        q = ops.blockfp8_dswiglu_quantize(h, dact, self.fmt_b, r.grad_block_scaling_dim, rowwise=want_y, colwise=want_t,
                                          want_colsum=colsum, amax_epsilon=r.fp8_quant_bwd_grad.amax_epsilon)
        return q[:2], q[2:4], q[4]

    def offer(self, handoff: DyHandoff, g: int, want_y: bool, want_t: bool) -> None:
        """Nothing: no DyHandoff producer has a block-scaled form.  RoPE backward and cross-entropy backward take their bf16 route
        and the Linear quantises the gradient it receives."""

    def taken(self, fp8, g: int):
        raise RuntimeError("Float8BlockScaling offers no DyHandoff, so no producer can have put FP8 copies into one")

    def quantize_weights(self, weights, ns, N: int, K: int, dev, g: int, want_t: bool):
        r = self.recipe
        fmt, dim, eps = self.fmt_f, r.w_block_scaling_dim, r.fp8_quant_fwd_weight.amax_epsilon
        ws_ = [(w if w.dtype == torch.bfloat16 else w.to(torch.bfloat16)).contiguous() for w in weights]
        if len(ws_) == 1:
            return ops.blockfp8_quantize(ws_[0], fmt, dim, rowwise=True, colwise=want_t, amax_epsilon=eps)
        if any(n % (128 if dim == 2 else 32) for n in ns):
            return ops.blockfp8_quantize(torch.cat(ws_, 0), fmt, dim, rowwise=True, colwise=want_t, amax_epsilon=eps)
        w8 = torch.empty((N, K), dtype=torch.uint8, device=dev)
        sc = torch.empty((K // 32, N), dtype=torch.uint8, device=dev)
        wt8 = torch.empty((K, N), dtype=torch.uint8, device=dev) if want_t else None
        sct = torch.empty((N // 32, K), dtype=torch.uint8, device=dev) if want_t else None
        o = 0
        for w, n in zip(ws_, ns):
            ops.blockfp8_quantize(w, fmt, dim, rowwise=True, colwise=want_t, amax_epsilon=eps,
                                  out=(w8[o:o + n], sc[:, o:o + n], wt8[:, o:o + n] if want_t else None,
                                       sct[o // 32:(o + n) // 32] if want_t else None))
            o += n
        return w8, sc, wt8, sct

    def new_sink(self, weights, ns, N: int, K: int, dev, g: int):
        return None


class _CurrentQ:
    __slots__ = ("recipe", "fmt_f", "fmt_b")
    mx = False
    cache_key, sink_key = "cs", "cssink"
    no_sink = ("Float8CurrentScaling keeps no optimiser-filled FP8 weight copies, which row-sharded weights (distributed.ShardedFP8DP, "
               "--sharding_mode fsdp_fp8) depend on: use --sharding_mode replicated (GradArenaDP) with this recipe")
    swiglu_adds_bias = True
    colsum_dtypes = None

    def __init__(self, recipe: Float8CurrentScaling, fmt_f: int, fmt_b: int):
        self.recipe, self.fmt_f, self.fmt_b = recipe, fmt_f, fmt_b

    @staticmethod
    def _triple(part, fmt: int, qp):
        return ops.current_scale(part, ops.FP8_MAX[fmt], qp.amax_epsilon, qp.power_2_scale)

    def quantize(self, x2, g: int, want_t: bool, norm=None):
        part = ops.amax_partial(x2.device, ops.amax_grid(*x2.shape))
        if norm is None:
            ops.amax_bf16(x2, part)
        else:
            ops.amax_norm(x2, norm[0], norm[1], part)
        t3 = self._triple(part, self.fmt_f, self.recipe.fp8_quant_fwd_inp)
        if norm is None:
            y, yT = ops.cast_amax(x2, t3[1:2], None, self.fmt_f, want_t=want_t)
        else:
            y, yT = ops.norm_cast(x2, norm[0], norm[1], t3[1:2], None, self.fmt_f, want_t=want_t)
        return (y, t3[2:3]), (yT, t3[2:3])

    def swiglu(self, h, g: int, want_t: bool, bias):
        part = ops.amax_partial(h.device, ops.amax_grid(h.shape[0], h.shape[1] // 2, 32))
        ops.amax_swiglu(h, bias, part)
        t3 = self._triple(part, self.fmt_f, self.recipe.fp8_quant_fwd_inp)
        y, yT = ops.swiglu_cast(h, t3[1:2], None, self.fmt_f, want_t=want_t, bias=bias)
        return (y, t3[2:3]), (yT, t3[2:3])

    def quantize_grad(self, g2, g: int, want_y: bool, want_t: bool, colsum: bool = False):
        part = ops.amax_partial(g2.device, ops.amax_grid(*g2.shape))
        ops.amax_bf16(g2, part)
        t3 = self._triple(part, self.fmt_b, self.recipe.fp8_quant_bwd_grad)
        out = ops.cast_amax(g2, t3[1:2], None, self.fmt_b, want_y=want_y, want_t=want_t, want_colsum=colsum)
        return (out[0], t3[2:3]), (out[1], t3[2:3]), out[2] if colsum else None

    def dswiglu(self, h, dact, g: int, want_y: bool, want_t: bool, colsum: bool, bias):
        part = ops.amax_partial(h.device, ops.amax_grid(h.shape[0], h.shape[1] // 2, 32))
        ops.amax_dswiglu(h, bias, dact, part)
        t3 = self._triple(part, self.fmt_b, self.recipe.fp8_quant_bwd_grad)
        y, yT, cs = ops.dswiglu_cast(h, dact, t3[1:2], None, self.fmt_b, want_y=want_y, want_t=want_t, want_colsum=colsum, bias=bias)
        return (y, t3[2:3]), (yT, t3[2:3]), cs

    def offer(self, handoff: DyHandoff, g: int, want_y: bool, want_t: bool) -> None:
        """Nothing: a DyHandoff producer needs the scale of grad_output before it has produced it.  RoPE backward and cross-entropy
        backward take their bf16 route and the Linear quantises the gradient it receives."""

    def taken(self, fp8, g: int):
        raise RuntimeError("Float8CurrentScaling offers no DyHandoff, so no producer can have put FP8 copies into one")

    operands = _DelayedQ.operands
    gemm = _DelayedQ.gemm
    unflat = _DelayedQ.unflat

    def quantize_weights(self, weights, ns, N: int, K: int, dev, g: int, want_t: bool):
        ws_ = [(w if w.dtype == torch.bfloat16 else w.to(torch.bfloat16)).contiguous() for w in weights]
        grids = [ops.amax_grid(n, K) for n in ns]
        part = ops.amax_partial(dev, sum(grids))
        o = 0
        for w, n in zip(ws_, grids):
            ops.amax_bf16(w, part[o:o + n])
            o += n
        t3 = self._triple(part, self.fmt_f, self.recipe.fp8_quant_fwd_weight)
        w8 = torch.empty((N, K), dtype=torch.uint8, device=dev)
        w8t = torch.empty((K, N), dtype=torch.uint8, device=dev) if want_t else None
        r = 0
        for w, n in zip(ws_, ns):
            ops.cast_amax(w, t3[1:2], None, self.fmt_f, y=w8[r:r + n], yT=None if w8t is None else w8t[:, r:r + n], want_t=want_t)
            r += n
        return w8, w8t, t3[2:3]

    def new_sink(self, weights, ns, N: int, K: int, dev, g: int):
        return None


def _weight_operand(spec: _GemmSpec, g: int, weights, ns, N: int, K: int, dev, need_t: bool):
    q, wc = spec.q, spec.wcache
    ck = (q.cache_key, g)
    if spec.first_mb is False and wc is not None:
        hit = wc.get(ck)
        if hit is not None:
            op = q.unflat(hit)
            if op[1][0] is not None or not need_t:
                return op
    keep = spec.first_mb is True and wc is not None
    shard = sharded_handle(weights)
    if shard is not None and (wc is None or spec.fmt_fwd != 0):
        raise RuntimeError("row-sharded weights need the module's FP8 weight cache and an E4M3 forward format")
    flat = None
    if wc is not None and spec.fmt_fwd == 0 and (weight_sinks_enabled() or shard is not None):
        sink = wc.get((q.sink_key, g))
        if sink is None or not sink.holds(weights, spec.meta_fwd):
            sink = None
            if (spec.training or shard is not None) and all(_weight_ok_for_sink(w, K) for w in weights):
                sink = q.new_sink(weights, ns, N, K, dev, g)
                if sink is not None:
                    wc[(q.sink_key, g)] = sink
        if shard is not None:
            if sink is None:
                raise RuntimeError(q.no_sink)
            shard.dp.wait_operand(sink)
            if not sink.fresh():
                q.refresh(shard.dp, sink)
        if sink is not None and sink.fresh():
            flat = q.sink_flat(sink, g)
    if flat is None:
        flat = q.quantize_weights(weights, ns, N, K, dev, g, need_t or keep)
    if keep:
        wc[ck] = flat
    return q.unflat(flat)


class _AddStatsFn(torch.autograd.Function):

    @staticmethod
    def forward(ctx, a, b, eps, bias=None):
        out, rstd = ops.add_rmsnorm_stats(a, b, eps, bias=bias)
        ctx.mark_non_differentiable(rstd)
        ctx.set_materialize_grads(False)
        return out, rstd

    @staticmethod
    def backward(ctx, dout, _drstd):
        return dout, dout, None, None


def residual_add_stats(a: torch.Tensor, b: torch.Tensor, eps: float, bias: Optional[torch.Tensor] = None):
    if (a.is_cuda and a.dtype == torch.bfloat16 and b.dtype == torch.bfloat16 and a.shape == b.shape and a.is_contiguous()
            and b.is_contiguous() and a.shape[-1] % 8 == 0 and (bias is None or a.shape[-1] == bias.numel())):
        bb = None if bias is None else bias.detach().to(torch.bfloat16).contiguous()
        return _AddStatsFn.apply(a, b, eps, bb)
    if bias is not None:
        b = b + bias.detach().to(b.dtype)
    return a + b, None


def _wgrad_out(weights, K: int) -> Optional[torch.Tensor]:
    shard = getattr(weights[0], "_mi_sharded", None)
    if shard is not None:
        return shard.dp.wgrad_buffer(weights, K)
    slot = getattr(weights[0], "_mi_grad_slot", None)
    if slot is None:
        return None
    arena, off = slot
    if arena.dtype != torch.bfloat16:
        return None
    end = off
    for w in weights:
        s = getattr(w, "_mi_grad_slot", None)
        if s is None or s[0] is not arena or s[1] != end or w.grad is not None or w.dtype != torch.bfloat16 or w.shape[1] != K:
            return None
        end += w.numel()
    return arena[off:end].view(-1, K)


def _grouped_or_two(q, grad, w_col, x_col, dw_out, need_dgrad: bool, need_wgrad: bool):
    dgrad, wgrad, mx, fmt_b, fmt_f = q.operands(grad[0], w_col), q.operands(grad[1], x_col), q.mx, q.fmt_b, q.fmt_f
    if need_dgrad and need_wgrad and ops.default_gemm_algo() in (0, 4, 47) and os.environ.get("LLM_FP8_AMD_NO_GROUPED_GEMM") != "1":
        g8, wt8 = dgrad[0], dgrad[2 if mx else 1]
        M, N = g8.shape
        K = wt8.shape[0]
        layout_ok = (all(t.is_contiguous() for t in dgrad + wgrad) if mx else
                     all(t.stride(1) == 1 for t in dgrad[:2] + wgrad[:2]))
        if ops.grouped_gemm_ok(((M, K, N), (N, K, M))) and layout_ok:
            dx = torch.empty((M, K), dtype=torch.bfloat16, device=g8.device)
            dw = dw_out if dw_out is not None else torch.empty((N, K), dtype=torch.bfloat16, device=g8.device)
            probs = [dgrad + (dx,), wgrad + (dw,)]
            cfg = ops.grouped_gemm_choice(probs, fmt_b, fmt_f, mx=mx)
            if cfg >= 0:
                (ops.gemm_mxfp8_grouped if mx else ops.gemm_fp8_grouped)(probs, fmt_b, fmt_f, tile_cfg=cfg)
                return dx, dw
    gemm = ops.gemm_mxfp8 if mx else ops.gemm_fp8
    dx = gemm(*dgrad, fmt_b, fmt_f) if need_dgrad else None
    dw = gemm(*wgrad, fmt_b, fmt_f, out=dw_out) if need_wgrad else None
    return dx, dw


def _skip_2d(dskip: Optional[torch.Tensor], like: torch.Tensor) -> Optional[torch.Tensor]:
    if dskip is None:
        return None
    d = dskip.reshape(like.shape)
    return d if (d.dtype == torch.bfloat16 and d.is_contiguous()) else d.to(torch.bfloat16).contiguous()


def _quantize_input(ctx, spec: _GemmSpec, x2, ln_w, want_t: bool, need_dgrad: bool):
    ctx.norm = None
    if ln_w is None:
        return spec.q.quantize(x2, spec.g, want_t)
    gam = (ln_w if ln_w.dtype == torch.bfloat16 else ln_w.to(torch.bfloat16)).contiguous()
    rstd = spec.rstd if spec.rstd is not None else ops.rmsnorm_stats(x2, spec.eps)
    if need_dgrad:
        ctx.norm = (x2, rstd, gam, ln_w.dtype)
    return spec.q.quantize(x2, spec.g, want_t, (rstd, gam))


def _finish_dx(ctx, dx, dskip, colsums=None):
    dln = None
    if ctx.norm is not None and dx is not None:
        xin, rstd, gam, ln_dtype = ctx.norm
        ctx.norm = None
        dx, dln = ops.rmsnorm_bwd(dx, xin, rstd, gam, dres=_skip_2d(dskip, dx), dgamma_dtype=ln_dtype, finish=colsums is None)
        dskip = None
        if colsums is not None:
            dln = (dln, ln_dtype)
    if colsums is not None:
        pend = [t for t in (*colsums, dln) if t is not None]
        if pend:
            done = iter(ops.colsum_finish_multi(pend))
            colsums = [None if t is None else next(done) for t in colsums]
            dln = None if dln is None else next(done)
    if ctx.spec.trigger_bwd_update:
        FP8GlobalStateManager.reduce_and_update_fp8_tensors(forward=False)
    if dx is not None:
        dx = dx.view(ctx.x_shape).to(ctx.x_dtype)
    if dskip is not None:
        dx = dskip if dx is None else dx + dskip
    return dx, dln, colsums


class _FP8LinearFn(torch.autograd.Function):

    @staticmethod
    def forward(ctx, x: torch.Tensor, bias: Optional[torch.Tensor], spec: _GemmSpec, ln_w: Optional[torch.Tensor],
                *weights: torch.Tensor):
        x2 = _as_bf16_2d(x)
        M, K = x2.shape
        if M % 8 or K % 16:
            raise RuntimeError(f"FP8 Linear needs tokens % 8 == 0 and in_features % 16 == 0, got {M} x {K}")
        ns = [w.shape[0] for w in weights]
        N = sum(ns)
        q, g = spec.q, spec.g
        need_dgrad = bool(ctx.needs_input_grad[0]) or bool(ctx.needs_input_grad[3])
        need_wgrad = any(ctx.needs_input_grad[4:])
        x8 = _quantize_input(ctx, spec, x2, ln_w, need_wgrad, need_dgrad)
        w8 = _weight_operand(spec, g, weights, ns, N, K, x2.device, need_dgrad)
        y = q.gemm(x8[0], w8[0], None if bias is None else bias.to(torch.bfloat16).contiguous())
        ctx.saved_fp8 = (x8[1], w8[1])
        if spec.dy_handoff is not None and bias is None and (need_wgrad or need_dgrad):
            q.offer(spec.dy_handoff, g, need_dgrad, need_wgrad)
        ctx.spec, ctx.ns, ctx.x_shape, ctx.x_dtype = spec, ns, x.shape, x.dtype
        ctx.w_dtypes = [w.dtype for w in weights]
        ctx.w_refs = weights if need_wgrad else None
        ctx.has_bias, ctx.bias_dtype = bias is not None, (None if bias is None else bias.dtype)
        ctx.need_wgrad, ctx.need_dgrad = need_wgrad, need_dgrad
        if spec.with_skip:
            ctx.set_materialize_grads(False)
            return y.view(*x.shape[:-1], N), x
        return y.view(*x.shape[:-1], N)

    @staticmethod
    def backward(ctx, dy: torch.Tensor, dskip: Optional[torch.Tensor] = None):
        spec = ctx.spec
        q, g = spec.q, spec.g
        g2 = _as_bf16_2d(dy)
        x_col, w_col = ctx.saved_fp8
        ctx.saved_fp8 = None
        db = None
        if spec.dy_handoff is not None and spec.dy_handoff.fp8 is not None:
            grad = q.taken(spec.dy_handoff.take(dy), g)
        elif ctx.has_bias and (q.colsum_dtypes is None or ctx.bias_dtype in q.colsum_dtypes):
            grad = q.quantize_grad(g2, g, ctx.need_dgrad, ctx.need_wgrad, colsum=True)
            db = ops.colsum_finish(grad[2], ctx.bias_dtype)
        else:
            grad = q.quantize_grad(g2, g, ctx.need_dgrad, ctx.need_wgrad)
        dx, dw = _grouped_or_two(q, grad, w_col, x_col, _wgrad_out(ctx.w_refs, x_col[0].shape[0]) if ctx.need_wgrad else None,
                                 ctx.need_dgrad, ctx.need_wgrad)
        if ctx.has_bias and db is None:
            db = g2.sum(0, dtype=torch.float32).to(ctx.bias_dtype)
        dx, dln, _ = _finish_dx(ctx, dx, dskip)
        dws: List[Optional[torch.Tensor]] = [None] * len(ctx.ns)
        if dw is not None:
            parts = torch.split(dw, ctx.ns, dim=0)
            dws = [p if p.dtype == dt else p.to(dt) for p, dt in zip(parts, ctx.w_dtypes)]
        return (dx, db, None, dln, *dws)


class _FP8SwiGLUMLPFn(torch.autograd.Function):

    @staticmethod
    def forward(ctx, x, w1, b1, w2, b2, spec: _GemmSpec, ln_w=None):
        x2 = _as_bf16_2d(x)
        M, K = x2.shape
        if M % 8 or K % 16:
            raise RuntimeError(f"FP8 LayerNormMLP needs tokens % 8 == 0 and hidden % 16 == 0, got {M} x {K}")
        q, dev = spec.q, x2.device
        need_dgrad = bool(ctx.needs_input_grad[0]) or bool(ctx.needs_input_grad[6])
        need_w = bool(ctx.needs_input_grad[1]) or bool(ctx.needs_input_grad[3])
        bwd = need_dgrad or need_w
        x8 = _quantize_input(ctx, spec, x2, ln_w, need_w, need_dgrad)
        w1_8 = _weight_operand(spec, 0, (w1,), [w1.shape[0]], w1.shape[0], K, dev, bwd)
        b1_bf = None if b1 is None else b1.detach().to(torch.bfloat16).contiguous()
        fuse_b1 = b1_bf is not None and q.swiglu_adds_bias and _FUSE_MLP_BIAS and (b1_bf.data_ptr() % 16 == 0)
        h = q.gemm(x8[0], w1_8[0], None if fuse_b1 else b1_bf)
        a8 = q.swiglu(h, 1, need_w, b1_bf if fuse_b1 else None)
        ctx.b1_fused = b1_bf if fuse_b1 else None
        w2_8 = _weight_operand(spec, 1, (w2,), [w2.shape[0]], w2.shape[0], w2.shape[1], dev, bwd)
        y = q.gemm(a8[0], w2_8[0], None if (b2 is None or spec.defer_bias) else b2.to(torch.bfloat16).contiguous())
        ctx.saved_fp8 = (x8[1], w1_8[1], a8[1], w2_8[1], h if bwd else None)
        ctx.spec, ctx.x_shape, ctx.x_dtype = spec, x.shape, x.dtype
        ctx.dtypes = (w1.dtype, None if b1 is None else b1.dtype, w2.dtype, None if b2 is None else b2.dtype)
        ctx.need_dgrad, ctx.need_w = need_dgrad, need_w
        ctx.w_refs = (w1, w2) if need_w else None
        if spec.with_skip:
            ctx.set_materialize_grads(False)
            return y.view(*x.shape[:-1], w2.shape[0]), x
        return y.view(*x.shape[:-1], w2.shape[0])

    @staticmethod
    def backward(ctx, dy, dskip=None):
        q = ctx.spec.q
        x_col, w1_col, a_col, w2_col, h = ctx.saved_fp8
        ctx.saved_fp8 = None
        dt_w1, dt_b1, dt_w2, dt_b2 = ctx.dtypes
        grad = q.quantize_grad(_as_bf16_2d(dy), 1, True, ctx.need_w, colsum=dt_b2 is not None)
        db2 = None if dt_b2 is None else (grad[2], dt_b2)
        dact, dw2 = _grouped_or_two(q, grad, w2_col, a_col, _wgrad_out(ctx.w_refs[1:], a_col[0].shape[0]) if ctx.need_w else None,
                                    True, ctx.need_w)
        grad = q.dswiglu(h, dact, 0, ctx.need_dgrad, ctx.need_w, dt_b1 is not None, ctx.b1_fused)
        db1 = None if dt_b1 is None else (grad[2], dt_b1)
        dx, dw1 = _grouped_or_two(q, grad, w1_col, x_col, _wgrad_out(ctx.w_refs[:1], x_col[0].shape[0]) if ctx.need_w else None,
                                  ctx.need_dgrad, ctx.need_w)
        dx, dln, (db1, db2) = _finish_dx(ctx, dx, dskip, (db1, db2))
        if dw1 is not None and dw1.dtype != dt_w1:
            dw1 = dw1.to(dt_w1)
        if dw2 is not None and dw2.dtype != dt_w2:
            dw2 = dw2.to(dt_w2)
        return dx, dw1, db1, dw2, db2, None, dln


class _FP8Module(torch.nn.Module):

    num_gemms = 1

    def __init__(self):
        super().__init__()
        self._meta_fwd: Optional[ModuleMeta] = None
        self._meta_bwd: Optional[ModuleMeta] = None
        self._meta_key = None
        self._pending_state = None
        self._wcache = {}
        self.default_is_first_microbatch = None

    def _spec(self, st, is_first_microbatch, g: int = 0, eps: float = 1e-5, **kw) -> _GemmSpec:
        recipe, mf, mb, first = st
        if is_first_microbatch is None:
            is_first_microbatch = self.default_is_first_microbatch
        return _GemmSpec(recipe, mf, mb, g, first and g == 0, self.training, eps, self._wcache, is_first_microbatch, **kw)

    def _norm(self, x):
        if self.normalization == "RMSNorm":
            return _rmsnorm(x, self.layer_norm_weight, self.eps, self.zero_centered_gamma)
        return _layernorm(x, self.layer_norm_weight, self.layer_norm_bias, self.eps, self.zero_centered_gamma)

    def _prepare(self, device) -> Optional[Tuple[Recipe, Optional[ModuleMeta], Optional[ModuleMeta], bool]]:
        if not FP8GlobalStateManager.is_fp8_enabled():
            return None
        recipe = FP8GlobalStateManager.get_fp8_recipe()
        first = FP8GlobalStateManager.is_first_fp8_module()
        if recipe.mxfp8() or recipe.current() or recipe.block():
            return recipe, None, None, first
        key = (recipe.fp8_format, recipe.amax_history_len, recipe.amax_compute_algo, recipe.margin, str(device))
        if self._meta_key != key:
            fa = FP8GlobalStateManager.arena(recipe, True, device)
            ba = FP8GlobalStateManager.arena(recipe, False, device)
            self._meta_fwd = ModuleMeta(fa, fa.alloc(3 * self.num_gemms), 3 * self.num_gemms)
            self._meta_bwd = ModuleMeta(ba, ba.alloc(2 * self.num_gemms), 2 * self.num_gemms)
            self._meta_key = key
            if self._pending_state is not None:
                self._meta_fwd.load_state(self._pending_state["fwd"])
                self._meta_bwd.load_state(self._pending_state["bwd"])
                self._pending_state = None
        else:
            FP8GlobalStateManager.arena(recipe, True, device)
            FP8GlobalStateManager.arena(recipe, False, device)
        return recipe, self._meta_fwd, self._meta_bwd, first

    def get_extra_state(self):
        if self._meta_fwd is None:
            return torch.empty(0, dtype=torch.uint8)
        buf = io.BytesIO()
        to_cpu = lambda d: {k: v.cpu() for k, v in d.items()}
        torch.save({"fwd": to_cpu(self._meta_fwd.state()), "bwd": to_cpu(self._meta_bwd.state())}, buf)
        return torch.frombuffer(bytearray(buf.getvalue()), dtype=torch.uint8)

    def set_extra_state(self, state):
        if state is None or (isinstance(state, torch.Tensor) and state.numel() == 0):
            return
        st = torch.load(io.BytesIO(state.cpu().numpy().tobytes()), weights_only=True)
        if self._meta_fwd is not None:
            self._meta_fwd.load_state(st["fwd"])
            self._meta_bwd.load_state(st["bwd"])
        else:
            self._pending_state = st


def _rmsnorm(x: torch.Tensor, weight: torch.Tensor, eps: float, zero_centered_gamma: bool = False) -> torch.Tensor:
    w = weight + 1 if zero_centered_gamma else weight
    return F.rms_norm(x, (x.shape[-1],), w, eps)


def _layernorm(x, weight, bias, eps, zero_centered_gamma=False):
    w = weight + 1 if zero_centered_gamma else weight
    return F.layer_norm(x, (x.shape[-1],), w, bias, eps)


class RMSNorm(torch.nn.Module):
    def __init__(self, hidden_size: int, eps: float = 1e-5, params_dtype=None, device="cuda", zero_centered_gamma=False):
        super().__init__()
        self.eps, self.zero_centered_gamma = eps, zero_centered_gamma
        self.weight = torch.nn.Parameter(torch.ones(hidden_size, dtype=params_dtype or torch.get_default_dtype(), device=device))

    def forward(self, x):
        return _rmsnorm(x, self.weight, self.eps, self.zero_centered_gamma)


class LayerNorm(torch.nn.Module):

    def __init__(self, hidden_size: int, eps: float = 1e-5, params_dtype=None, device="cuda", zero_centered_gamma=False):
        super().__init__()
        self.eps, self.zero_centered_gamma = eps, zero_centered_gamma
        dt = params_dtype or torch.get_default_dtype()
        self.weight = torch.nn.Parameter(torch.ones(hidden_size, dtype=dt, device=device))
        self.bias = torch.nn.Parameter(torch.zeros(hidden_size, dtype=dt, device=device))

    def forward(self, x):
        return _layernorm(x, self.weight, self.bias, self.eps, self.zero_centered_gamma)


def _init_weight(shape, dtype, device, init_method=None):
    w = torch.empty(shape, dtype=dtype, device=device)
    if init_method is not None:
        init_method(w)
    else:
        torch.nn.init.normal_(w, mean=0.0, std=0.023)
    return torch.nn.Parameter(w)


class Linear(_FP8Module):

    def __init__(self, in_features: int, out_features: int, bias: bool = True, params_dtype=None, device="cuda",
                 init_method=None, **_ignored):
        super().__init__()
        self.in_features, self.out_features = in_features, out_features
        dt = params_dtype or torch.get_default_dtype()
        self.weight = _init_weight((out_features, in_features), dt, device, init_method)
        self.bias = torch.nn.Parameter(torch.zeros(out_features, dtype=dt, device=device)) if bias else None
        self.use_bias = bias

    def forward(self, inp: torch.Tensor, is_first_microbatch=None) -> torch.Tensor:
        st = self._prepare(inp.device)
        if st is None:
            if getattr(self, "_pending_norm", None) is not None:
                raise RuntimeError("Linear: a deferred RMSNorm is pending but FP8 is off for this forward")
            return F.linear(inp, _master(self.weight).to(inp.dtype), None if self.bias is None else self.bias.to(inp.dtype))
        handoff = DyHandoff() if (getattr(self, "offer_dy_handoff", False) and self.training and torch.is_grad_enabled()
                                  and self.bias is None) else None
        pn, self._pending_norm = getattr(self, "_pending_norm", None), None
        ln_w, eps, rstd = None, 1e-5, None
        if pn is not None:
            ln_w, eps, rs, ptr, shape = pn
            if inp.data_ptr() != ptr or tuple(inp.shape) != shape:
# ... 157 lines not shown
```

### llm_fp8_amd/pytorch/ops.py

```python
from __future__ import annotations

import ctypes
import os
from typing import Optional, Tuple

import torch

from .. import _lib
from .profiler import KernelTimer

E4M3, E5M2 = _lib.MI_FMT_E4M3, _lib.MI_FMT_E5M2
FP8_MAX = {E4M3: 448.0, E5M2: 57344.0}


_SK_WORKSPACE = {}


def ensure_gemm_workspace(device: torch.device) -> None:
    idx = device.index if device.index is not None else torch.cuda.current_device()
    if idx in _SK_WORKSPACE:
        return
    lib = _lib.load()
    with torch.cuda.device(idx):
        nbytes = int(lib.mi_gemm_workspace_bytes())
        ws = torch.zeros(nbytes, dtype=torch.uint8, device=torch.device("cuda", idx))
        torch.cuda.synchronize(idx)
        _lib.check(lib.mi_gemm_set_workspace(ws.data_ptr(), nbytes), "mi_gemm_set_workspace")
    _SK_WORKSPACE[idx] = ws


def default_gemm_algo() -> int:
    env = os.environ.get("LLM_FP8_AMD_GEMM_ALGO")
    if env is not None:
        return int(env)
    d = torch.distributed
    if d.is_available() and d.is_initialized() and d.get_world_size() > 1:
        return 5
    return 47 if os.environ.get("LLM_FP8_AMD_GEMM_W4", "1") != "0" else 0


def _stream() -> int:
    return torch.cuda.current_stream().cuda_stream


def _dev(*ts):
    for t in ts:
        if t is not None and not t.is_cuda:
            raise RuntimeError("llm_fp8_amd ops need device (HIP) tensors; there is no CPU fallback")


def _ptr(t: Optional[torch.Tensor]) -> Optional[int]:
    return None if t is None else t.data_ptr()


def colsum_finish(partial: torch.Tensor, dtype: torch.dtype = torch.bfloat16) -> torch.Tensor:
    _dev(partial)
    assert partial.dtype == torch.float32 and partial.dim() == 2 and partial.is_contiguous()
    P, C = partial.shape
    if dtype not in (torch.bfloat16, torch.float32):
        return partial.sum(0).to(dtype)
    out = torch.empty(C, dtype=dtype, device=partial.device)
    _lib.check(_lib.load().mi_colsum_finish(partial.data_ptr(), P, C, out.data_ptr(), 0 if dtype == torch.bfloat16 else 1, _stream()),
               "mi_colsum_finish")
    return out


def colsum_finish_multi(items):
    import ctypes
    outs = [None] * len(items)
    todo = []
    for i, (partial, dtype) in enumerate(items):
        _dev(partial)
        assert partial.dtype == torch.float32 and partial.dim() == 2 and partial.is_contiguous()
        if dtype not in (torch.bfloat16, torch.float32):
            outs[i] = partial.sum(0).to(dtype)
        else:
            outs[i] = torch.empty(partial.shape[1], dtype=dtype, device=partial.device)
            todo.append(i)
    for k in range(0, len(todo), 4):
        grp = todo[k:k + 4]
        n = len(grp)
        parts = (ctypes.c_void_p * n)(*[items[i][0].data_ptr() for i in grp])
        Ps = (ctypes.c_int64 * n)(*[items[i][0].shape[0] for i in grp])
        Cs = (ctypes.c_int64 * n)(*[items[i][0].shape[1] for i in grp])
        os_ = (ctypes.c_void_p * n)(*[outs[i].data_ptr() for i in grp])
        dts = (ctypes.c_int * n)(*[0 if items[i][1] == torch.bfloat16 else 1 for i in grp])
        _lib.check(_lib.load().mi_colsum_finish_multi(parts, Ps, Cs, os_, dts, n, _stream()), "mi_colsum_finish_multi")
    return outs


def cast_amax(x: torch.Tensor, scale: torch.Tensor, amax: Optional[torch.Tensor], fmt: int,
              want_y: bool = True, want_t: bool = True,
              y: Optional[torch.Tensor] = None, yT: Optional[torch.Tensor] = None, want_colsum: bool = False):
    _dev(x, scale, amax, y, yT)
    assert x.dtype == torch.bfloat16 and x.dim() == 2 and x.is_contiguous()
    assert scale.dtype == torch.float32 and (amax is None or amax.dtype == torch.float32)
    R, C = x.shape
    if want_y and y is None:
        y = torch.empty((R, C), dtype=torch.uint8, device=x.device)
    if want_t and yT is None:
        yT = torch.empty((C, R), dtype=torch.uint8, device=x.device)
    if y is not None:
        assert y.dtype == torch.uint8 and y.shape == (R, C) and y.stride(1) == 1
    if yT is not None:
        assert yT.dtype == torch.uint8 and yT.shape == (C, R) and yT.stride(1) == 1
    cs = torch.empty(((R + 63) // 64, C), dtype=torch.float32, device=x.device) if want_colsum else None
    tail = (R, C, y.stride(0) if y is not None else C, yT.stride(0) if yT is not None else R, fmt, _stream())
    head = (x.data_ptr(), _ptr(y), _ptr(yT), scale.data_ptr(), _ptr(amax))
    fn = _lib.load().mi_cast_amax_colsum if want_colsum else _lib.load().mi_cast_amax
    args = head + ((cs.data_ptr(),) if want_colsum else ()) + tail
    t = KernelTimer.active
    if t is None:
        rc = fn(*args)
    else:
        nb = R * C * (2 + (y is not None) + (yT is not None))
        with t.span("cast_amax", f"{R}x{C}", float(R * C), float(nb)):
            rc = fn(*args)
    _lib.check(rc, "mi_cast_amax")
    return (y, yT, cs) if want_colsum else (y, yT)


AMAX_MAX_PARTIALS = 1024
_AMAX_PARTIAL: dict = {}
_CU_COUNT: dict = {}


def amax_grid(rows: int, cols: int, tile_rows: int = 64) -> int:
    idx = torch.cuda.current_device()
    if idx not in _CU_COUNT:
        _CU_COUNT[idx] = int(torch.cuda.get_device_properties(idx).multi_processor_count) or 256
    tiles = -(-rows // tile_rows) * -(-cols // 64)
    return max(1, min(-(-tiles // 4), 2 * _CU_COUNT[idx], AMAX_MAX_PARTIALS))


def amax_partial(device: torch.device, n: int) -> torch.Tensor:
    idx = device.index if device.index is not None else torch.cuda.current_device()
    buf = _AMAX_PARTIAL.get(idx)
    if buf is None or buf.numel() < n:
        buf = _AMAX_PARTIAL[idx] = torch.empty(max(n, 4 * AMAX_MAX_PARTIALS), dtype=torch.float32, device=torch.device("cuda", idx))
    return buf[:n]


def _amax_call(name: str, args, label: str, elems: float, nbytes: float) -> None:
    fn = _lib.require(name, "Float8CurrentScaling")
    t = KernelTimer.active
    if t is None:
        rc = fn(*args)
    else:
        with t.span("amax", label, elems, nbytes):
            rc = fn(*args)
    _lib.check(rc, name)


def _partial_ok(partial: torch.Tensor) -> int:
    _dev(partial)
    assert partial.dtype == torch.float32 and partial.dim() == 1 and partial.is_contiguous() and 1 <= partial.numel() <= AMAX_MAX_PARTIALS
    return partial.numel()


def amax_bf16(x: torch.Tensor, partial: torch.Tensor) -> None:
    _dev(x)
    assert x.dtype == torch.bfloat16 and x.dim() == 2 and x.is_contiguous()
    R, C = x.shape
    _amax_call("mi_amax_bf16", (x.data_ptr(), partial.data_ptr(), _partial_ok(partial), R, C, _stream()), f"{R}x{C}", float(R * C),
               2.0 * R * C)


def amax_norm(x: torch.Tensor, rstd: torch.Tensor, gamma: torch.Tensor, partial: torch.Tensor) -> None:
    _dev(x, rstd, gamma)
    assert x.dtype == torch.bfloat16 and gamma.dtype == torch.bfloat16 and x.dim() == 2 and x.is_contiguous() and gamma.is_contiguous()
    assert rstd.dtype == torch.float32 and rstd.is_contiguous() and rstd.numel() == x.shape[0] and gamma.numel() == x.shape[1]
    R, C = x.shape
    _amax_call("mi_amax_norm", (x.data_ptr(), rstd.data_ptr(), gamma.data_ptr(), partial.data_ptr(), _partial_ok(partial), R, C, _stream()),
               f"norm {R}x{C}", float(R * C), 2.0 * R * C)


def amax_swiglu(h: torch.Tensor, bias: Optional[torch.Tensor], partial: torch.Tensor) -> None:
    _dev(h, bias)
    assert h.dtype == torch.bfloat16 and h.dim() == 2 and h.is_contiguous() and h.shape[1] % 2 == 0
    R, F = h.shape[0], h.shape[1] // 2
    assert bias is None or (bias.dtype == torch.bfloat16 and bias.numel() == 2 * F and bias.is_contiguous())
    _amax_call("mi_amax_swiglu", (h.data_ptr(), _ptr(bias), partial.data_ptr(), _partial_ok(partial), R, F, _stream()),
               f"swiglu {R}x{F}", float(R * F), 4.0 * R * F)


def amax_dswiglu(h: torch.Tensor, bias: Optional[torch.Tensor], dact: torch.Tensor, partial: torch.Tensor) -> None:
    _dev(h, bias, dact)
    assert h.dtype == torch.bfloat16 and dact.dtype == torch.bfloat16 and h.dim() == 2 and h.is_contiguous() and dact.is_contiguous()
    R, F = h.shape[0], h.shape[1] // 2
    assert dact.shape == (R, F) and (bias is None or (bias.dtype == torch.bfloat16 and bias.numel() == 2 * F and bias.is_contiguous()))
    _amax_call("mi_amax_dswiglu", (h.data_ptr(), _ptr(bias), dact.data_ptr(), partial.data_ptr(), _partial_ok(partial), R, F, _stream()),
               f"dswiglu {R}x{F}", float(2 * R * F), 6.0 * R * F)


def current_scale(partial: torch.Tensor, fp8_max: float, amax_epsilon: float = 0.0, pow2: bool = False) -> torch.Tensor:
    _dev(partial)
    assert partial.dtype == torch.float32 and partial.dim() == 1 and partial.is_contiguous() and partial.numel() >= 1
    out3 = torch.empty(3, dtype=torch.float32, device=partial.device)
    fn = _lib.require("mi_current_scale", "Float8CurrentScaling")
    _lib.check(fn(partial.data_ptr(), partial.numel(), float(fp8_max), float(amax_epsilon), int(bool(pow2)), out3.data_ptr(), _stream()),
               "mi_current_scale")
    return out3


def scale_update(amax_history: torch.Tensor, scale: torch.Tensor, scale_inv: torch.Tensor,
                 fp8_max: torch.Tensor, margin: int = 0, algo: str = "max") -> None:
    _dev(amax_history, scale, scale_inv, fp8_max)
    assert amax_history.dim() == 2 and amax_history.stride(1) == 1 and amax_history.dtype == torch.float32
    H, S = amax_history.shape
    assert scale.numel() == S and scale_inv.numel() == S and fp8_max.numel() == S
    assert scale.is_contiguous() and scale_inv.is_contiguous() and fp8_max.is_contiguous()
    rc = _lib.load().mi_scale_update(amax_history.data_ptr(), scale.data_ptr(), scale_inv.data_ptr(),
                                     fp8_max.data_ptr(), H, S, amax_history.stride(0), margin,
                                     0 if algo == "max" else 1, _stream())
    _lib.check(rc, "mi_scale_update")


def _default_algo_for(M: int, N: int, K: int, out: Optional[torch.Tensor], out_dtype: torch.dtype, mx: bool) -> int:
    algo = default_gemm_algo()
    bf16 = out_dtype == torch.bfloat16 and (out is None or out.dtype == torch.bfloat16)
    if ((mx and algo not in (0, 1, 4, 5)) or (algo == 3 and (M % 256 or N % 256 or K % 128)) or (algo == 47 and not bf16)
            or (algo == 5 and ((M % 256 and M % 192) or (N % 256 and N % 192) or K % 256 or not bf16))):
        return 0
    return algo


def gemm_fp8(a8: torch.Tensor, b8: torch.Tensor, sa_inv: torch.Tensor, sb_inv: torch.Tensor,
             fmt_a: int, fmt_b: int, bias: Optional[torch.Tensor] = None,
             out: Optional[torch.Tensor] = None, out_dtype: torch.dtype = torch.bfloat16,
             algo: Optional[int] = None) -> torch.Tensor:
    if algo is None:
        algo = _default_algo_for(a8.shape[0], b8.shape[0], a8.shape[1], out, out_dtype, mx=False)
    _dev(a8, b8, sa_inv, sb_inv, bias, out)
    if algo == 44:
        ensure_gemm_workspace(a8.device)
    assert a8.dtype == torch.uint8 and b8.dtype == torch.uint8 and a8.dim() == 2 and b8.dim() == 2
    assert a8.stride(1) == 1 and b8.stride(1) == 1
    M, K = a8.shape
    N, K2 = b8.shape
    assert K == K2, f"contraction mismatch {K} vs {K2}"
    if out is None:
        out = torch.empty((M, N), dtype=out_dtype, device=a8.device)
    assert out.shape == (M, N) and out.stride(1) == 1 and out.dtype in (torch.bfloat16, torch.float32)
    if bias is not None:
        assert bias.dtype == torch.bfloat16 and bias.numel() == N and bias.is_contiguous()
    args = (a8.data_ptr(), b8.data_ptr(), out.data_ptr(), sa_inv.data_ptr(), sb_inv.data_ptr(), _ptr(bias), M, N, K,
            a8.stride(0), b8.stride(0), out.stride(0), fmt_a, fmt_b, 0 if out.dtype == torch.bfloat16 else 1, algo,
            _stream())
    t = KernelTimer.active
    if t is None:
        rc = _lib.load().mi_gemm_fp8(*args)
    else:
        with t.span("gemm_fp8", f"{M}x{N}x{K}", 2.0 * M * N * K, M * K + N * K + out.element_size() * M * N):
            rc = _lib.load().mi_gemm_fp8(*args)
    _lib.check(rc, "mi_gemm_fp8")
    return out


def mxfp8_quantize(x: torch.Tensor, fmt: int = E4M3, rowwise: bool = True, colwise: bool = True, out=None,
                   want_colsum: bool = False):
    _dev(x)
    assert x.dtype == torch.bfloat16 and x.dim() == 2 and x.is_contiguous()
    R, C = x.shape
    y_row = s_row = y_colT = s_colT = None
    ld = R
    if out is not None:
        y_row, s_row, y_colT, s_colT = out
        _dev(y_row, s_row, y_colT, s_colT)
        assert (y_row is not None) == rowwise and (y_colT is not None) == colwise
        if rowwise:
            assert y_row.shape == (R, C) and y_row.is_contiguous() and s_row.shape == (C // 32, R) and s_row.stride(1) == 1
            ld = s_row.stride(0)
        if colwise:
            assert y_colT.shape == (C, R) and y_colT.stride(1) == 1 and s_colT.shape == (R // 32, C) and s_colT.is_contiguous()
            assert not rowwise or y_colT.stride(0) == ld
            ld = y_colT.stride(0)
    else:
        if rowwise:
            y_row = torch.empty((R, C), dtype=torch.uint8, device=x.device)
            s_row = torch.empty((C // 32, R), dtype=torch.uint8, device=x.device)
        if colwise:
            y_colT = torch.empty((C, R), dtype=torch.uint8, device=x.device)
            s_colT = torch.empty((R // 32, C), dtype=torch.uint8, device=x.device)
    cs = torch.empty(((R + 127) // 128, C), dtype=torch.float32, device=x.device) if want_colsum else None
    if out is None and not want_colsum:
        fn, args = _lib.load().mi_mxfp8_quantize, (x.data_ptr(), _ptr(y_row), _ptr(s_row), _ptr(y_colT), _ptr(s_colT), R, C, fmt, _stream())
    else:
        fn, args = _lib.load().mi_mxfp8_quantize_ex, (x.data_ptr(), _ptr(y_row), _ptr(s_row), _ptr(y_colT), _ptr(s_colT), _ptr(cs),
                                                      R, C, ld, fmt, _stream())
    t = KernelTimer.active
    if t is None:
        rc = fn(*args)
    else:
        nb = R * C * (2 + (1 + 1 / 32) * (int(rowwise) + int(colwise)))
        with t.span("mxfp8_quantize", f"{R}x{C}", float(R * C), float(nb)):
            rc = fn(*args)
    _lib.check(rc, "mi_mxfp8_quantize")
    return (y_row, s_row, y_colT, s_colT, cs) if want_colsum else (y_row, s_row, y_colT, s_colT)


def gemm_mxfp8(a8, sa, b8, sb, fmt_a: int = E4M3, fmt_b: int = E4M3, bias=None, out=None,
               out_dtype: torch.dtype = torch.bfloat16, algo: Optional[int] = None) -> torch.Tensor:
    _dev(a8, sa, b8, sb, bias, out)
    if algo is None:
        algo = _default_algo_for(a8.shape[0], b8.shape[0], a8.shape[1], out, out_dtype, mx=True)
    if algo == 44:
        ensure_gemm_workspace(a8.device)
    M, K = a8.shape
    N, K2 = b8.shape
    assert K == K2 and a8.is_contiguous() and b8.is_contiguous() and sa.is_contiguous() and sb.is_contiguous()
    assert sa.shape == (K // 32, M) and sb.shape == (K // 32, N), "scales must be block-major [K/32, rows]"
    if out is None:
        out = torch.empty((M, N), dtype=out_dtype, device=a8.device)
    assert out.is_contiguous() and out.shape == (M, N)
    args = (a8.data_ptr(), sa.data_ptr(), b8.data_ptr(), sb.data_ptr(), out.data_ptr(), _ptr(bias), M, N, K, fmt_a,
            fmt_b, 0 if out.dtype == torch.bfloat16 else 1, algo, _stream())
    t = KernelTimer.active
    if t is None:
        rc = _lib.load().mi_gemm_mxfp8(*args)
    else:
        with t.span("gemm_mxfp8", f"{M}x{N}x{K}", 2.0 * M * N * K, M * K + N * K + out.element_size() * M * N):
            rc = _lib.load().mi_gemm_mxfp8(*args)
    _lib.check(rc, "mi_gemm_mxfp8")
    return out


def rope_qkv_forward(qkv: torch.Tensor, cos: torch.Tensor, sin: torch.Tensor, n_q: int, n_kv: int, head_dim: int, seq: int):
    _dev(qkv, cos, sin)
    assert qkv.dtype == torch.bfloat16 and qkv.is_contiguous() and qkv.dim() == 2
    T, W = qkv.shape
    assert W == (n_q + 2 * n_kv) * head_dim and cos.dtype == torch.float32 and cos.shape[-1] == head_dim // 2 and cos.shape[0] >= seq
    q = torch.empty((T, n_q * head_dim), dtype=torch.bfloat16, device=qkv.device)
    k = torch.empty((T, n_kv * head_dim), dtype=torch.bfloat16, device=qkv.device)
    v = torch.empty((T, n_kv * head_dim), dtype=torch.bfloat16, device=qkv.device)
    rc = _lib.load().mi_rope_qkv(qkv.data_ptr(), q.data_ptr(), k.data_ptr(), v.data_ptr(), cos.data_ptr(), sin.data_ptr(),
                                 T, seq, n_q, n_kv, head_dim, 0, _stream())
    _lib.check(rc, "mi_rope_qkv")
    return q, k, v


def rope_qkv_backward(dq: torch.Tensor, dk: torch.Tensor, dv: torch.Tensor, cos: torch.Tensor, sin: torch.Tensor,
                      n_q: int, n_kv: int, head_dim: int, seq: int) -> torch.Tensor:
    _dev(dq, dk, dv, cos, sin)
    dq, dk, dv = (t.contiguous() for t in (dq, dk, dv))
    T = dq.shape[0]
    out = torch.empty((T, (n_q + 2 * n_kv) * head_dim), dtype=torch.bfloat16, device=dq.device)
    rc = _lib.load().mi_rope_qkv(out.data_ptr(), dq.data_ptr(), dk.data_ptr(), dv.data_ptr(), cos.data_ptr(), sin.data_ptr(),
                                 T, seq, n_q, n_kv, head_dim, 1, _stream())
    _lib.check(rc, "mi_rope_qkv")
    return out


def mxfp8_rope_bwd_quantize(dq: torch.Tensor, dk: torch.Tensor, dv: torch.Tensor, cos: torch.Tensor, sin: torch.Tensor, n_q: int,
                            n_kv: int, head_dim: int, seq: int, fmt: int, rowwise: bool = True, colwise: bool = True):
    _dev(dq, dk, dv, cos, sin)
    dq, dk, dv = (t.contiguous() for t in (dq, dk, dv))
    T, W = dq.shape[0], (n_q + 2 * n_kv) * head_dim
    y_row = s_row = y_colT = s_colT = None
    if rowwise:
        y_row = torch.empty((T, W), dtype=torch.uint8, device=dq.device)
        s_row = torch.empty((W // 32, T), dtype=torch.uint8, device=dq.device)
    if colwise:
        y_colT = torch.empty((W, T), dtype=torch.uint8, device=dq.device)
        s_colT = torch.empty((T // 32, W), dtype=torch.uint8, device=dq.device)
    args = (dq.data_ptr(), dk.data_ptr(), dv.data_ptr(), cos.data_ptr(), sin.data_ptr(), _ptr(y_row), _ptr(s_row), _ptr(y_colT),
            _ptr(s_colT), T, seq, n_q, n_kv, head_dim, fmt, _stream())
    t = KernelTimer.active
    if t is None:
        rc = _lib.load().mi_mxfp8_rope_bwd_quantize(*args)
    else:
        with t.span("mxfp8_quantize", f"rope {T}x{W}", float(T * W), float(T * W * (2 + (1 + 1 / 32) * (int(rowwise) + int(colwise))))):
            rc = _lib.load().mi_mxfp8_rope_bwd_quantize(*args)
    _lib.check(rc, "mi_mxfp8_rope_bwd_quantize")
    return y_row, s_row, y_colT, s_colT


def _group_shapes(problems, mx: bool):
    ib = 2 if mx else 1
    return tuple((p[0].shape[0], p[ib].shape[0], p[0].shape[1]) for p in problems)


def _grouped_launch(entry: str, span: str, arr, shapes, fmt_a: int, fmt_b: int, tile_cfg: int) -> None:
    fn = getattr(_lib.load(), entry)
    args = (ctypes.byref(arr), len(shapes), fmt_a, fmt_b, tile_cfg, _stream())
    t = KernelTimer.active
    if t is None:
        rc = fn(*args)
    else:
        work = sum(2.0 * M * N * K for M, N, K in shapes)
        nbytes = sum(M * K + N * K + 2 * M * N for M, N, K in shapes)
        with t.span(span, "+".join(f"{M}x{N}x{K}" for M, N, K in shapes), work, nbytes):
            rc = fn(*args)
    _lib.check(rc, entry)


def gemm_fp8_grouped(problems, fmt_a: int, fmt_b: int, tile_cfg: int = -1) -> None:
    arr = (_lib.GemmProblem * len(problems))()
    for i, (a8, b8, sa, sb, out) in enumerate(problems):
        _dev(a8, b8, sa, sb, out)
        assert a8.dtype == torch.uint8 and b8.dtype == torch.uint8 and out.dtype == torch.bfloat16
        assert a8.stride(1) == 1 and b8.stride(1) == 1 and out.stride(1) == 1 and a8.shape[1] == b8.shape[1]
        assert out.shape == (a8.shape[0], b8.shape[0])
        arr[i] = _lib.GemmProblem(a8.data_ptr(), b8.data_ptr(), out.data_ptr(), sa.data_ptr(), sb.data_ptr(), a8.shape[0], b8.shape[0],
                                  a8.shape[1], a8.stride(0), b8.stride(0), out.stride(0))
    _grouped_launch("mi_gemm_fp8_grouped", "gemm_fp8", arr, _group_shapes(problems, False), fmt_a, fmt_b, tile_cfg)


def gemm_mxfp8_grouped(problems, fmt_a: int, fmt_b: int, tile_cfg: int = -1) -> None:
    arr = (_lib.GemmMxProblem * len(problems))()
    for i, (a8, sa, b8, sb, out) in enumerate(problems):
        _dev(a8, sa, b8, sb, out)
        M, K = a8.shape
        N, K2 = b8.shape
        assert a8.dtype == torch.uint8 and b8.dtype == torch.uint8 and out.dtype == torch.bfloat16
        assert K == K2 and a8.is_contiguous() and b8.is_contiguous() and sa.is_contiguous() and sb.is_contiguous()
        assert sa.shape == (K // 32, M) and sb.shape == (K // 32, N), "scales must be block-major [K/32, rows]"
        assert out.is_contiguous() and out.shape == (M, N)
        arr[i] = _lib.GemmMxProblem(a8.data_ptr(), sa.data_ptr(), b8.data_ptr(), sb.data_ptr(), out.data_ptr(), M, N, K)
    _grouped_launch("mi_gemm_mxfp8_grouped", "gemm_mxfp8", arr, _group_shapes(problems, True), fmt_a, fmt_b, tile_cfg)


def grouped_gemm_ok(shapes, strides_ok: bool = True) -> bool:
    if not strides_ok or not shapes or len(shapes) > 4:
        return False
    if not any(all(M % bm == 0 and N % bn == 0 for M, N, K in shapes) for bm, bn in _TILE_CFGS):
        return False
    if any(K % 256 or M * K >= 2 ** 31 or N * K >= 2 ** 31 or M * N * 2 >= 2 ** 31 for M, N, K in shapes):
        return False
    return True


_TILE_CFGS = ((256, 256), (256, 192), (192, 256), (192, 192))
_TILE_EFF = (1.0, 0.90, 0.90, 0.80)
_GROUP_PLAN: dict = {}


def grouped_gemm_plan(shapes, n_cu: int = 256) -> int:
    key = (tuple(shapes), n_cu)
    if key in _GROUP_PLAN:
        return _GROUP_PLAN[key]
    import heapq
    best = -1
    if grouped_gemm_ok(shapes):
        fixed = 4.0
        sep = 0.0
        for M, N, K in shapes:
            c = min((-(-((M // bm) * (N // bn)) // n_cu)) * (K // 128) * (bm * bn / 65536.0) / eff
                    for (bm, bn), eff in zip(_TILE_CFGS, _TILE_EFF) if M % bm == 0 and N % bn == 0)
            sep += c + fixed
        best_cost = None
        for cfg, ((bm, bn), eff) in enumerate(zip(_TILE_CFGS, _TILE_EFF)):
            if any(M % bm or N % bn for M, N, K in shapes):
                continue
            probs = sorted(((K // 128, (M // bm) * (N // bn)) for M, N, K in shapes), reverse=True)
            total = sum(t for _, t in probs)
            g = min(total, n_cu)
            loads = [(0, v) for v in range(g)]
            heapq.heapify(loads)
            per_wg = [0] * g
            for nk, tiles in probs:
                for _ in range(tiles):
                    load, v = heapq.heappop(loads)
                    per_wg[v] += 1
                    heapq.heappush(loads, (load + nk, v))
            if max(per_wg) > 64:
                continue
            cost = max(l for l, _ in loads) * (bm * bn / 65536.0) / eff * 1.02 + fixed
            if best_cost is None or cost < best_cost:
                best_cost, best = cost, cfg
        if best_cost is None or best_cost >= 0.98 * sep:
            best = -1
    _GROUP_PLAN[key] = best
    return best


_GROUP_TUNED: dict = {}


def grouped_gemm_choice(problems, fmt_a: int, fmt_b: int, mx: bool = False) -> int:
    mode = os.environ.get("LLM_FP8_AMD_GROUPED_GEMM", "auto")
    if mode == "off":
        return -1
    if mode == "auto":
        import torch.distributed as dist
        mode = "plan" if (dist.is_available() and dist.is_initialized()) else "autotune"
    if mode == "plan":
        return grouped_gemm_plan(_group_shapes(problems, mx))
    if mode != "autotune":
        raise ValueError(f"LLM_FP8_AMD_GROUPED_GEMM={mode!r}: expected auto, plan, autotune or off")
    return grouped_gemm_autotune(problems, fmt_a, fmt_b, mx=mx)


def _tuned_key(shapes, fmt_a: int, fmt_b: int, mx: bool):
    return ("mx", tuple(shapes), fmt_a, fmt_b) if mx else (tuple(shapes), fmt_a, fmt_b)


def grouped_gemm_autotune(problems, fmt_a: int, fmt_b: int, iters: int = 5, mx: bool = False) -> int:
    shapes = _group_shapes(problems, mx)
    key = _tuned_key(shapes, fmt_a, fmt_b, mx)
    hit = _GROUP_TUNED.get(key)
    if hit is not None:
        return hit
    single, grouped = (gemm_mxfp8, gemm_mxfp8_grouped) if mx else (gemm_fp8, gemm_fp8_grouped)
    problems = [(*p[:4], torch.empty_like(p[4])) for p in problems]
    cands = [-1]
    if grouped_gemm_ok(shapes):
        cands += [cfg for cfg, (bm, bn) in enumerate(_TILE_CFGS) if all(M % bm == 0 and N % bn == 0 for M, N, K in shapes)]
        if (not mx and all(M % 256 == 0 and N % 256 == 0 and K >= 512 for M, N, K in shapes)
                and os.environ.get("LLM_FP8_AMD_GEMM_W4G", "1") != "0"):
            cands.append(4)

    def run(c):
        if c == -1:
            for p in problems:
                single(*p[:4], fmt_a, fmt_b, out=p[4])
        else:
            grouped(problems, fmt_a, fmt_b, tile_cfg=c)

    saved, KernelTimer.active = KernelTimer.active, None
    try:
        live = []
        for c in cands:
            try:
                run(c)
# ... 390 lines not shown
```

Baseline: 88780 tokens/s.

## Add 256x192 tile variant of persistent W4 GEMM and select it by cost model

Adds a 256x192 output-tile form of the persistent wave-specialised FP8 GEMM kernel. It has its own compile-time-checked phase, DMA and epilogue schedule, a smaller B buffer in LDS, and narrow-row store handling. A new default algo 39 runs the existing 47 selection logic and then switches to the 192-wide tile when a rounds-times-efficiency cost model predicts it beats the 256x256 or P8 choice. The aim is better wave quantisation across CUs for N dimensions divisible by 192, such as Llama-3.2-3B's 3072 and 8192 dims. In exchange the tile does less MFMA work per LDS byte, and the heuristic efficiency constants may pick it in the wrong cases.

```diff
diff --git a/llm_fp8_amd/csrc/mi_gemm.hip b/llm_fp8_amd/csrc/mi_gemm.hip
--- a/llm_fp8_amd/csrc/mi_gemm.hip
+++ b/llm_fp8_amd/csrc/mi_gemm.hip
@@ -1020,7 +1020,7 @@
 }
 
 
-static int pick_tile_cfg(int64_t M, int64_t N, int64_t K) {
+static int pick_tile_cfg(int64_t M, int64_t N, int64_t K, double* cost_out = nullptr) {
   const double cold = 1.0 + 1150.0 / (double)(K > 0 ? K : 1);
   const double eff[4] = {1.0, 0.88 / cold, 0.92, 0.80 / cold};
   const int ncu = num_cus();
@@ -1036,7 +1036,20 @@
       best_cost = cost;
     }
   }
+  if (cost_out) *cost_out = best_cost;
   return best;
+}
+
+static bool w4_tile192_wins(int64_t M, int64_t N, int64_t K, bool w4_256) {
+  const double k = (double)(K > 0 ? K : 1);
+  const double eff_192 = 0.955 / (1.0 + 460.0 / k), eff_256 = 1.163 / (1.0 + 679.0 / k);
+  const int ncu = num_cus();
+  auto rounds = [&](int64_t tiles) { return (double)((tiles + ncu - 1) / ncu); };
+  const double cost_192 = rounds((M / 256) * (N / 192)) * 256 * 192 / eff_192;
+  double cost_47 = 0;
+  if (w4_256) cost_47 = rounds((M / 256) * (N / 256)) * 256 * 256 / eff_256;
+  else if (pick_tile_cfg(M, N, K, &cost_47) < 0) return false;
+  return cost_192 < cost_47 * 0.98;
 }
 
 struct SkWorkspace {
@@ -1065,7 +1078,7 @@
   return U >= nk ? (int)U : 0;
 }
 
-enum ShapeClass { kAnyShape, kFastOk, kP8Ok, kP8Ok256 };
+enum ShapeClass { kAnyShape, kFastOk, kP8Ok, kP8Ok256, kP8OkN192 };
 constexpr int kPick = -1;
 constexpr int kCfgById = -2;
 constexpr int kNoBuild = -1;
@@ -1091,6 +1104,7 @@
     {7, 8,   kFamW4,      1,  0, 0,        1, 1, kP8Ok256,  0, kBiasRefused, 0},
     {9, 9,   kFamW4P,     0,  0, 0,        0, 0, kP8Ok256,  0, kBiasAdded,   0},
     {10, 12, kFamW4P,     1,  0, 0,        0, 1, kP8Ok256,  0, kBiasRefused, 1},
+    {49, 49, kFamW4P,     0,  0, 1,        0, 0, kP8OkN192, 0, kBiasAdded,   0},
     {13, 14, kFam8Phase,  1,  0, kPick,    0, 1, kFastOk,   0, kBiasAdded,   0},
     {15, 15, kFamP8,      1,  0, kPick,    0, 1, kP8Ok,     0, kBiasUnused,  1},
     {16, 22, kFamP8,      3,  0, kPick,    0, 1, kP8Ok,     0, kBiasUnused,  1},
@@ -1105,6 +1119,8 @@
     {66, 68, kFamW4,      0,  4, 0,        1, 1, kP8Ok256,  0, kBiasUnused,  1},
     {50, 69, kFamW4, kNoBuild, 0, 0,       1, 1, kP8Ok256,  0, kBiasUnused,  1},
     {70, 73, kFamW4P,     4,  0, 0,        0, 1, kP8Ok256,  0, kBiasUnused,  1},
+    {74, 76, kFamW4P,     1,  0, 1,        0, 1, kP8OkN192, 0, kBiasUnused,  1},
+    {77, 77, kFamW4P,     7,  0, 1,        0, 1, kP8OkN192, 0, kBiasUnused,  1},
 };
 
 #ifdef MI_DIAG
@@ -1140,10 +1156,14 @@
   const bool p8_ok = (M % 256 == 0 || M % 192 == 0) && (N % 256 == 0 || N % 192 == 0) && K > 0 && (K % (2 * BK) == 0) &&
                      out == 0 && M * lda < (1LL << 31) && N * ldb < (1LL << 31) && M * ldd * 2 < (1LL << 31);
   const bool p8_ok_256 = p8_ok && M % 256 == 0 && N % 256 == 0;
+  const bool p8_ok_n192 = p8_ok && M % 256 == 0 && N % 192 == 0;
   const int ncu = num_cus();
   const int64_t tiles_256 = (M / 256) * (N / 256);
-  if (algo == 47) {
+  if (algo == 47 || algo == 39) {
+    const bool with_192 = algo == 39 && !mx;
     algo = (p8_ok_256 && K >= 512 && pick_tile_cfg(M, N, K) == 0 && (tiles_256 + ncu - 1) / ncu <= 64) ? 9 : 0;
+    if (with_192 && p8_ok_n192 && K >= 512 && ((M / 256) * (N / 192) + ncu - 1) / ncu <= 64 && w4_tile192_wins(M, N, K, algo == 9))
+      algo = 49;
   }
   if (algo == 0) algo = p8_ok ? 4 : ((fast_ok && !mx) ? 3 : 1);
   MI_CHECK_SHAPE(entry != kEntryClock || algo == 4 || algo == 9, "mi_gemm_fp8_clock: the shape does not run on a persistent kernel");
@@ -1151,10 +1171,11 @@
   MI_CHECK_ARG(r == nullptr || !r->lab || kLabLibrary,
                "%s: algo %d is a timing / diagnostic build; it lives in the lab library (make -C llm_fp8_amd/csrc lab)", kWho[entry], algo);
   MI_CHECK_ARG(r != nullptr, "%s: unknown algo %d", kWho[entry], algo);
-  const bool shape_ok[] = {true, fast_ok, p8_ok, p8_ok_256};
+  const bool shape_ok[] = {true, fast_ok, p8_ok, p8_ok_256, p8_ok_n192};
   static const char* const kNeeds[] = {"", "M,N % 256 == 0 and K % 128 == 0",
                                        "M,N % 256 (or 192) == 0, K % 256 == 0, bf16 output, operands < 2 GiB",
-                                       "M,N,K % 256 == 0, bf16 output, operands < 2 GiB"};
+                                       "M,N,K % 256 == 0, bf16 output, operands < 2 GiB",
+                                       "M % 256 == 0, N % 192 == 0, K % 256 == 0, bf16 output, operands < 2 GiB"};
   MI_CHECK_SHAPE(shape_ok[r->shape], "%s: algo %d needs %s", kWho[entry], algo, kNeeds[r->shape]);
   p.algo = algo;
   p.family = r->family;
@@ -1212,13 +1233,16 @@
       MI_CHECK_ARG(e4m3 || !r->e4m3_only, "mi_gemm (w4): variant %d is a timing build of the lab library", w4_number);
       MI_CHECK_ARG(p.build != kNoBuild, "mi_gemm (w4): no such schedule variant %d", w4_number);
       break;
-    case kFamW4P:
-      p.grid_x = (int)(tiles_256 < ncu ? tiles_256 : ncu);
-      MI_CHECK_SHAPE((tiles_256 + p.grid_x - 1) / p.grid_x <= 64 && K >= 512 && M / 256 < 16384 && N / 256 < 16384,
+    case kFamW4P: {
+      p.tiles_n = (int)(N / kTileBn[p.tile_cfg]);
+      const int64_t tiles = (int64_t)p.tiles_m * p.tiles_n;
+      p.grid_x = (int)(tiles < ncu ? tiles : ncu);
+      MI_CHECK_SHAPE((tiles + p.grid_x - 1) / p.grid_x <= 64 && K >= 512 && p.tiles_m < 16384 && p.tiles_n < 16384,
                      "mi_gemm (w4 persistent): needs K >= 512, at most 64 tiles per workgroup and fewer than 16384 tiles per dimension");
       MI_CHECK_ARG(e4m3 || p.build != 2, "mi_gemm (w4): the clock-stamp build is E4M3 x E4M3 only");
       MI_CHECK_ARG(e4m3 || !r->e4m3_only, "mi_gemm (w4): timing variant %d is built for E4M3 x E4M3 only", w4_number);
       break;
+    }
   }
   return MI_OK;
 }
diff --git a/llm_fp8_amd/csrc/mi_gemm_w4.hip b/llm_fp8_amd/csrc/mi_gemm_w4.hip
--- a/llm_fp8_amd/csrc/mi_gemm_w4.hip
+++ b/llm_fp8_amd/csrc/mi_gemm_w4.hip
@@ -260,6 +260,55 @@
   return kFrameSlots <= 160;
 }
 static_assert(schedule_ok(), "epilogue schedule violates a deadline");
+
+namespace n192 {
+constexpr int kKtSlots = 48;
+constexpr int phase_begin(int G) { return (G >> 2) * kKtSlots + ((G & 3) == 0 ? 0 : (G & 3) == 1 ? 16 : (G & 3) == 2 ? 24 : 32); }
+constexpr int phase_len(int P) { return (P == 1 || P == 2) ? 8 : 16; }
+constexpr bool wide(int r) { return r < 4 || r >= 12; }
+constexpr int conv_len(int r) { return wide(r) ? 5 : 2;  }
+constexpr int conv_start(int r) { return r < 4 ? 19 + 8 * r : r < 8 ? 51 + 3 * (r - 4) : r < 12 ? 63 + 2 * (r - 8) : 71 + 5 * (r - 12); }
+constexpr int kStores = 24;
+constexpr int store_slot(int e) { return 24 + 4 * e; }
+constexpr int store_row(int e) { return e < 8 ? e >> 1 : e < 16 ? e - 4 : 12 + ((e - 16) >> 1); }
+constexpr int store_half(int e) { return (e < 8 || e >= 16) ? (e & 1) : 0; }
+constexpr int first_store(int r) { return r < 4 ? 2 * r : r < 12 ? r + 4 : 16 + 2 * (r - 12); }
+constexpr int last_store(int r) { return wide(r) ? first_store(r) + 1 : first_store(r); }
+constexpr int kFrameSlots = store_slot(kStores - 1) + 4;
+constexpr int wait_x(int G) {
+  const int lo = phase_begin(G < 5 ? 0 : G - 5), hi = phase_begin(G);
+  int n = 0;
+  for (int e = 0; e < kStores; ++e)
+    if (store_slot(e) >= lo && store_slot(e) < hi) ++n;
+  return n;
+}
+constexpr int dma_in_phase(int P) { return (P & 3) == 2 ? 2 : 4; }
+constexpr int wait_dma(int P) {
+  int n = 0;
+  for (int q = P + 3; q < P + 8; ++q) n += dma_in_phase(q);
+  return n;
+}
+constexpr int reads_in_phase(int P) { return (P & 3) == 0 ? 4 : 8; }
+constexpr int final_slot(int r, int j) {
+  const int q = r >> 2, i = r & 3;
+  return phase_begin(q) + (wide(r) ? 4 * i + j : 2 * i + j);
+}
+constexpr bool schedule_ok() {
+  for (int r = 0; r < 16; ++r) {
+    for (int j = 0; j < (wide(r) ? 4 : 2); ++j) {
+      if (conv_start(r) + j < final_slot(r, j) + 3) return false;
+      if (conv_start(r) + j >= kKtSlots + final_slot(r, j)) return false;
+    }
+    if (r > 0 && conv_start(r) < conv_start(r - 1) + conv_len(r - 1)) return false;
+    if (store_slot(first_store(r)) < conv_start(r) + conv_len(r)) return false;
+    if (store_row(first_store(r)) != r || store_row(last_store(r)) != r) return false;
+    if (r + kPark < 16 && conv_start(r + kPark) + 1 <= store_slot(last_store(r)) + 3) return false;
+  }
+  return kFrameSlots <= 3 * kKtSlots && kFrameSlots <= phase_begin(11);
+}
+static_assert(schedule_ok(), "epilogue schedule of the 256 x 192 tile violates a deadline");
+static_assert(wait_dma(0) == 18 && wait_dma(1) == 18 && wait_dma(2) == 18 && wait_dma(3) == 16, "stage sizes 4, 4, 2, 4");
+}
 }
 
 template <int FA, int FB>
@@ -280,13 +329,19 @@
   int K, lda, ldb, ldd, tiles_m, tiles_n, a_bytes, b_bytes, d_bytes, n_cols;
 };
 
-template <int FA, int FB, int ABL, int MODE>
+template <int FA, int FB, int ABL, int MODE, int T192 = 0>
 __global__ __launch_bounds__(256, 1) void gemm_w4p(const std::conditional_t<MODE == 2, GroupArgs, W4Single> ka) {
   constexpr bool GROUPED = MODE == 2, BIAS = MODE == 1;
+  static_assert(!(GROUPED && T192), "the grouped form walks 256 x 256 tiles only");
+  constexpr int NJ1 = T192 ? 2 : 4;
+  constexpr int kBufB = T192 ? 56 * 1024 : kBufBytes;
+  constexpr int kLdsB = 2 * kBufB;
+  constexpr int kBnT = T192 ? 192 : 256;
+  constexpr int kKtSlots = T192 ? w4::n192::kKtSlots : 64, kFrame = T192 ? w4::n192::kFrameSlots : w4::kFrameSlots;
   constexpr int S = 3;
   static_assert(w4::sched_lag(S) == 2, "the cursor logic below assumes every stage of step s goes to step s + 2");
   static_assert(!(GROUPED && ABL != 0), "the grouped form has no timing builds");
-  __shared__ __attribute__((aligned(16))) uint8_t lds[kLdsBytes + (ABL == 7 ? 8192 : 0)];
+  __shared__ __attribute__((aligned(16))) uint8_t lds[kLdsB + (ABL == 7 ? 8192 : 0)];
   int stamp_idx = 0;
   const int tid = threadIdx.x, lane = tid & 63;
   const int wave = __builtin_amdgcn_readfirstlane(tid >> 6);
@@ -348,11 +403,11 @@
     const int t = __builtin_amdgcn_readlane(tab, ti);
     p = (t >> 28) & 3;
     ra = (t & 0x3FFF) * 256;
-    rb = ((t >> 14) & 0x3FFF) * 256;
+    rb = ((t >> 14) & 0x3FFF) * kBnT;
   };
 
   uint8_t* const buf0 = lds;
-  uint8_t* const buf1 = lds + kBufBytes;
+  uint8_t* const buf1 = lds + kBufB;
   auto dma = [&](rsrc_t rs, uint8_t* dst_base, int voff, int soff, auto p_c) __attribute__((always_inline)) {
     constexpr int IMM = decltype(p_c)::value * 1024;
     __builtin_amdgcn_raw_ptr_buffer_load_lds(rs, LDS_PTR(dst_base), 16, voff, soff - IMM, IMM, 0);
@@ -412,7 +467,12 @@
   };
   auto stage_b = [&](int h, const cursor_t& c, uint8_t* buf, auto p_c) __attribute__((always_inline)) {
     constexpr int p = decltype(p_c)::value;
-    dma(c.rsB, buf + (h ? kOffB1 : kOffB0) + wave * 4096, c.b_v, c.ob + c.kb + (h * 64 + p * 8) * c.ldb, p_c);
+    if constexpr (T192) {
+      if (h) dma(c.rsB, buf + kOffB1 + wave * 2048, c.b_v, c.ob + c.kb + (128 - 16 * wave + p * 8) * c.ldb, p_c);
+      else dma(c.rsB, buf + kOffB0 + wave * 4096, c.b_v, c.ob + c.kb + (p * 8) * c.ldb, p_c);
+    } else {
+      dma(c.rsB, buf + (h ? kOffB1 : kOffB0) + wave * 4096, c.b_v, c.ob + c.kb + (h * 64 + p * 8) * c.ldb, p_c);
+    }
   };
 
   int fa_lo[2], fa_hi[2], fb_lo[2], fb_hi[2];
@@ -423,16 +483,17 @@
     const int l0 = (int)(size_t)LDS_PTR(lds);
 #pragma unroll
     for (int b = 0; b < 2; ++b) {
-      fa_lo[b] = l0 + b * kBufBytes + kOffA0 + wr * 4 * 2048 + flo;
-      fa_hi[b] = l0 + b * kBufBytes + kOffA0 + wr * 4 * 2048 + fhi;
-      fb_lo[b] = l0 + b * kBufBytes + kOffB0 + wc * 4 * 2048 + flo;
-      fb_hi[b] = l0 + b * kBufBytes + kOffB0 + wc * 4 * 2048 + fhi;
+      fa_lo[b] = l0 + b * kBufB + kOffA0 + wr * 4 * 2048 + flo;
+      fa_hi[b] = l0 + b * kBufB + kOffA0 + wr * 4 * 2048 + fhi;
+      fb_lo[b] = l0 + b * kBufB + kOffB0 + wc * 4 * 2048 + flo;
+      fb_hi[b] = l0 + b * kBufB + kOffB0 + wc * 4 * 2048 + fhi;
     }
   }
   typedef const __attribute__((address_space(3))) v4i* lds_v4i_p;
-  auto read_part = [&](v8i (&dst)[4], int lo, int hi, int half, int n) __attribute__((always_inline)) {
+  const int b1_adj = T192 ? -wc * 2 * 2048 : 0;
+  auto read_part = [&](v8i (&dst)[4], int lo, int hi, int half, int n, int adj = 0) __attribute__((always_inline)) {
     const int f = n >> 1;
-    const v4i v = *reinterpret_cast<lds_v4i_p>((size_t)(unsigned)(((n & 1) ? hi : lo) + half * kHalfBytes + f * 2048));
+    const v4i v = *reinterpret_cast<lds_v4i_p>((size_t)(unsigned)(((n & 1) ? hi : lo) + adj + half * kHalfBytes + f * 2048));
     if (n & 1) dst[f].hi = v;
     else dst[f].lo = v;
   };
@@ -455,6 +516,11 @@
     int d_off, ldd, d_voff;
     float alpha;
   };
+  int d_voff_h = 0;
+  if constexpr (T192) {
+    const int fr = lane & 15, fq = lane >> 4;
+    d_voff_h = ((wr * 128 + fr) * ka.ldd + 128 + wc * 32 + (fq & 1) * 16 + (fq >> 1) * 8) * 2;
+  }
   auto epi_of = [&](int ti, bool real) __attribute__((always_inline)) -> epi_t {
     int p, ra, rb;
     tile_of(ti, p, ra, rb);
@@ -479,7 +545,7 @@
     asm volatile("v_mov_b32 %0, %1" : "=v"(ln) : "v"(lane));
     const int fr = ln & 15, fq = ln >> 4;
     const int ecol = (fq & 1) * 16 + (fq >> 1) * 8;
-    e.d_voff = ((wr * 128 + (fr & 7)) * e.ldd + wc * 128 + (fr >> 3) * 32 + ecol) * 2;
+    e.d_voff = ((wr * 128 + (fr & 7)) * e.ldd + wc * (T192 ? 64 : 128) + (fr >> 3) * 32 + ecol) * 2;
     return e;
   };
   v4i park[w4::kPark][2];
@@ -530,16 +596,19 @@
     }
   };
   auto store_event = [&](auto e_c, auto w_c, const epi_t& e) __attribute__((always_inline)) {
-    constexpr int ev = decltype(e_c)::value, r = ev >> 1, half = ev & 1, w = decltype(w_c)::value;
+    constexpr int ev = decltype(e_c)::value, w = decltype(w_c)::value;
+    constexpr int r = T192 ? w4::n192::store_row(ev) : ev >> 1, half = T192 ? w4::n192::store_half(ev) : ev & 1;
+    constexpr bool NARROW = T192 && !w4::n192::wide(r);
     constexpr int q = r >> 2, a = q >> 1, b = (q == 1 || q == 2) ? 1 : 0, i = r & 3;
-    const int rowoff = e.d_off + ((a * 64 + i * 16 + half * 8) * e.ldd + b * 64) * 2;
+    const int rowoff = e.d_off + ((a * 64 + i * 16 + half * 8) * e.ldd + (NARROW ? 0 : b * 64)) * 2;
+    const int voff = NARROW ? d_voff_h : e.d_voff;
     const v4i data = park[r % w4::kPark][half];
     if (ABL == 1) {
       asm volatile("" ::"v"(data));
     } else {
       constexpr int kAux = ABL == 4 ? 0 : ABL == 5 ? 2 : ABL == 6 ? 18 : 16;
       if (wave == w) {
-        __builtin_amdgcn_raw_buffer_store_b128((mi::v4u)data, e.rs, e.d_voff, rowoff, kAux);
+        __builtin_amdgcn_raw_buffer_store_b128((mi::v4u)data, e.rs, voff, rowoff, kAux);
         asm volatile("s_nop 1" ::"v"(data) : "memory");
       }
     }
@@ -548,10 +617,12 @@
     constexpr int g = decltype(g_c)::value;
     if constexpr (ABL != 3) {
       static_for<16>([&](auto r_c) __attribute__((always_inline)) {
-        constexpr int r = decltype(r_c)::value, cs = w4::conv_start(r);
-        if constexpr (g >= cs && g < cs + 5) conv_chunk(r_c, std::integral_constant<int, g - cs>{}, e);
+        constexpr int r = decltype(r_c)::value, cs = T192 ? w4::n192::conv_start(r) : w4::conv_start(r);
+        constexpr int len = T192 ? w4::n192::conv_len(r) : 5;
+        if constexpr (g >= cs && g < cs + len) conv_chunk(r_c, std::integral_constant<int, g - cs>{}, e);
       });
-      if constexpr (g >= w4::store_slot(0) && g < w4::kFrameSlots)
+      static_assert(w4::n192::store_slot(0) == w4::store_slot(0), "both tile shapes deal store event e to slot 24 + 4 e + wave");
+      if constexpr (g >= w4::store_slot(0) && g < kFrame)
         store_event(std::integral_constant<int, (g - w4::store_slot(0)) / 4>{}, std::integral_constant<int, (g - w4::store_slot(0)) % 4>{}, e);
     }
   };
@@ -559,6 +630,16 @@
   if constexpr (BIAS) rsBias = __builtin_amdgcn_make_buffer_rsrc((void*)ka.bias, 0, ka.n_cols * 2, 0x00020000);
   auto load_bias = [&](int rb) __attribute__((always_inline)) {
     if constexpr (BIAS) {
+      if constexpr (T192) {
+        const int voff = (wc * 32 + (lane >> 4) * 4) * 2;
+#pragma unroll
+        for (int b = 0; b < 2; ++b)
+#pragma unroll
+          for (int j = 0; j < (b ? NJ1 : 4); ++j)
+            bias_w[b][j] = __builtin_bit_cast(
+                v2u_, __builtin_amdgcn_raw_buffer_load_b64(rsBias, voff, rb * 2 + (b ? 128 + j * 16 : wc * 32 + j * 16) * 2, 0));
+        return;
+      }
       const int voff = (wc * 128 + (lane >> 4) * 4) * 2;
 #pragma unroll
       for (int b = 0; b < 2; ++b)
@@ -575,27 +656,32 @@
     constexpr bool ZC = MODE_ == w4::FIRST;
     constexpr bool NOST = ABL == 1 || ABL == 3;
     constexpr int G_ = MODE_ + P;
-    constexpr int XB = (BIAS && MODE_ != w4::MID && G_ >= 9 && G_ <= 13) ? 8 : 0;
-    constexpr int X = ((NOST || MODE_ == w4::MID) ? 0 : w4::wait_x(G_)) + XB;
-    static_assert(20 + X <= 63, "vmcnt is a 6-bit counter");
+    constexpr int XB = (BIAS && MODE_ != w4::MID && G_ >= 9 && G_ <= 13) ? (T192 ? 4 + NJ1 : 8) : 0;
+    constexpr int X = ((NOST || MODE_ == w4::MID) ? 0 : T192 ? w4::n192::wait_x(G_) : w4::wait_x(G_)) + XB;
+    constexpr int LEN = T192 ? w4::n192::phase_len(P) : 16, NJ = LEN / 4;
+    constexpr int ND = T192 ? w4::n192::dma_in_phase(P) : 4, NR = T192 ? w4::n192::reads_in_phase(P) : 8;
+    constexpr int VM = T192 ? w4::n192::wait_dma(P) : 20;
+    constexpr int LGKM = T192 ? w4::n192::reads_in_phase((P + 3) & 3) : 8;
+    constexpr int G0 = T192 ? (MODE_ == w4::MID ? 0 : w4::n192::phase_begin(G_)) : 16 * G_;
+    static_assert(VM + X <= 63, "vmcnt is a 6-bit counter");
     __builtin_amdgcn_sched_barrier(0);
-    static_for<16>([&](auto k_c) __attribute__((always_inline)) {
-      constexpr int k = decltype(k_c)::value, i = k >> 2, j = k & 3;
+    static_for<LEN>([&](auto k_c) __attribute__((always_inline)) {
+      constexpr int k = decltype(k_c)::value, i = k / NJ, j = k % NJ;
       if constexpr (ZC) mfma_acc_zero<FA, FB>(af[i], bf[j], c[i][j], unit);
       else mfma_acc<FA, FB>(af[i], bf[j], c[i][j], unit);
       if constexpr (k == w4::sched_kb(S)) {
         __builtin_amdgcn_sched_barrier(0);
-        asm volatile("s_waitcnt vmcnt(%0) lgkmcnt(8)" ::"n"(20 + X) : "memory");
+        asm volatile("s_waitcnt vmcnt(%0) lgkmcnt(%1)" ::"n"(VM + X), "n"(LGKM) : "memory");
         __builtin_amdgcn_s_barrier();
         if constexpr (BIAS && MODE_ == w4::SECOND && P == 0) load_bias(rb_cur);
       }
-      static_for<4>([&](auto p_c) __attribute__((always_inline)) {
-        if constexpr (k == w4::sched_dm(S, decltype(p_c)::value)) stage(p_c);
+      static_for<ND>([&](auto p_c) __attribute__((always_inline)) {
+        if constexpr (k == (LEN == 8 ? 1 + 2 * decltype(p_c)::value : w4::sched_dm(S, decltype(p_c)::value))) stage(p_c);
       });
 #pragma unroll
-      for (int n = 0; n < 8; ++n)
-        if (k == w4::sched_rd(S, n)) read(n);
-      if constexpr (MODE_ != w4::MID && MODE_ != w4::THIRD) epi_slot(std::integral_constant<int, 16 * (MODE_ + P) + k>{}, e);
+      for (int n = 0; n < NR; ++n)
+        if (k == (LEN == 8 ? n : w4::sched_rd(S, n))) read(n);
+      if constexpr (MODE_ != w4::MID && MODE_ != w4::THIRD) epi_slot(std::integral_constant<int, G0 + k>{}, e);
       __builtin_amdgcn_sched_barrier(0);
     });
   };
@@ -610,12 +696,15 @@
     if (ABL == 7) {
       if (bid == 0 && wave == 0 && stamp_idx < 1024) {
         const unsigned long long t = __builtin_amdgcn_s_memtime();
-        if (lane == 0) reinterpret_cast<unsigned long long*>(lds + kLdsBytes)[stamp_idx] = t;
+        if (lane == 0) reinterpret_cast<unsigned long long*>(lds + kLdsB)[stamp_idx] = t;
       }
       ++stamp_idx;
     }
     phase(mode_c, p0_t{}, aA, b0[par], acc[0][0], [&](auto p) __attribute__((always_inline)) { stage_a(0, c2, cur, p); },
-          [&](int n) __attribute__((always_inline)) { read_part(b1, fb_lo[par], fb_hi[par], 1, n); }, e, rb_cur);
+          [&](int n) __attribute__((always_inline)) {
+            if constexpr (T192) read_part(b1, fb_lo[par], fb_hi[par], 1, n, b1_adj);
+            else read_part(b1, fb_lo[par], fb_hi[par], 1, n);
+          }, e, rb_cur);
     phase(mode_c, p1_t{}, aA, b1, acc[0][1], [&](auto p) __attribute__((always_inline)) { stage_b(0, c2, cur, p); },
           [&](int n) __attribute__((always_inline)) { read_part(aB, fa_lo[par], fa_hi[par], 1, n); }, e, rb_cur);
     phase(mode_c, p2_t{}, aB, b1, acc[1][1], [&](auto p) __attribute__((always_inline)) { stage_b(1, c2, cur, p); },
@@ -642,7 +731,7 @@
     const int lr = lane >> 3, chunk = ((lane & 7) ^ swz_f(lr)) * 16;
     const int row = (wave >> 1) * 128 + (wave & 1) * 32 + lr;
     c2.a_v = row * ka.lda + chunk;
-    c2.b_v = row * ka.ldb + chunk;
+    c2.b_v = (T192 ? wave * 32 + lr : row) * ka.ldb + chunk;
     total = my_tiles * c2.nk;
   }
   enter_tile(c2, 0);
@@ -652,19 +741,22 @@
   auto stage4b = [&](int h, uint8_t* buf) __attribute__((always_inline)) {
     static_for<4>([&](auto p_c) __attribute__((always_inline)) { stage_b(h, c2, buf, p_c); });
   };
+  auto stage_b1 = [&](uint8_t* buf) __attribute__((always_inline)) {
+    static_for<NJ1>([&](auto p_c) __attribute__((always_inline)) { stage_b(1, c2, buf, p_c); });
+  };
   stage4a(0, buf0);
   stage4b(0, buf0);
-  stage4b(1, buf0);
+  stage_b1(buf0);
   stage4a(1, buf0);
   advance(c2);
   stage4a(0, buf1);
   stage4b(0, buf1);
-  asm volatile("s_waitcnt vmcnt(20)" ::: "memory");
+  asm volatile("s_waitcnt vmcnt(%0)" ::"n"(16 + NJ1) : "memory");
   __builtin_amdgcn_s_barrier();
-  stage4b(1, buf1);
+  stage_b1(buf1);
 #pragma unroll
   for (int n = 0; n < 8; ++n) read_part(aA, fa_lo[0], fa_hi[0], 0, n);
-  asm volatile("s_waitcnt vmcnt(20)" ::: "memory");
+  asm volatile("s_waitcnt vmcnt(%0)" ::"n"(12 + 2 * NJ1) : "memory");
   __builtin_amdgcn_s_barrier();
   stage4a(1, buf1);
 #pragma unroll
@@ -729,13 +821,13 @@
       if (bid == 0 && wave == 0) {
         asm volatile("s_waitcnt lgkmcnt(0)" ::: "memory");
         for (int i = lane; i < 1024; i += 64)
-          ka.dbg[i] = i < stamp_idx ? reinterpret_cast<unsigned long long*>(lds + kLdsBytes)[i] : (i == stamp_idx ? t_end : 0ull);
+          ka.dbg[i] = i < stamp_idx ? reinterpret_cast<unsigned long long*>(lds + kLdsB)[i] : (i == stamp_idx ? t_end : 0ull);
       }
     }
   }
   asm volatile("s_waitcnt vmcnt(0) lgkmcnt(0)\n\ts_nop 7\n\ts_nop 7" ::: "memory");
-  static_for<w4::kFrameSlots - 64>([&](auto g_c) __attribute__((always_inline)) {
-    epi_slot(std::integral_constant<int, 64 + decltype(g_c)::value>{}, ep_prev);
+  static_for<kFrame - kKtSlots>([&](auto g_c) __attribute__((always_inline)) {
+    epi_slot(std::integral_constant<int, kKtSlots + decltype(g_c)::value>{}, ep_prev);
     __builtin_amdgcn_sched_barrier(0);
   });
 }
@@ -743,9 +835,11 @@
 #ifdef MI_DIAG
 #define MI_W4_BUILDS(X) X(0, 0) X(1, 0) X(2, 0) X(0, 1) X(1, 1) X(2, 1) X(0, 3) X(1, 3) X(2, 3) X(0, 4) X(1, 4) X(2, 4)
 #define MI_W4P_BUILDS_E4M3(X) X(1) X(2) X(3) X(4) X(5) X(6) X(7)
+#define MI_W4P192_BUILDS_E4M3(X) X(1) X(2) X(3) X(7)
 #else
 #define MI_W4_BUILDS(X) X(0, 0)
 #define MI_W4P_BUILDS_E4M3(X) X(2)
+#define MI_W4P192_BUILDS_E4M3(X)
 #endif
 
 int launch_w4(const GemmPlan& p, const GemmArgs& g) {
@@ -775,6 +869,17 @@
       ws.a_bytes = (int)(g.M * g.lda); ws.b_bytes = (int)(g.N * g.ldb); ws.d_bytes = (int)(g.M * g.ldd * 2); ws.n_cols = (int)g.N;
       if (p.build != 0 && (FA != 0 || FB != 0)) MI_NOT_COMPILED(p);
 #define MI_W4P(ABLv) case ABLv: hipLaunchKernelGGL((gemm_w4p<0, 0, ABLv, 0>), grid, block, 0, g.st, ws); break;
+#define MI_W4P192(ABLv) case ABLv: hipLaunchKernelGGL((gemm_w4p<0, 0, ABLv, 0, 1>), grid, block, 0, g.st, ws); break;
+      if (p.tile_cfg == 1) {
+        switch (p.build) {
+          case 0:
+            if (ws.bias) hipLaunchKernelGGL((gemm_w4p<FA, FB, 0, 1, 1>), grid, block, 0, g.st, ws);
+            else hipLaunchKernelGGL((gemm_w4p<FA, FB, 0, 0, 1>), grid, block, 0, g.st, ws);
+            break;
+          MI_W4P192_BUILDS_E4M3(MI_W4P192)
+          default: MI_NOT_COMPILED(p);
+        }
+      } else
       switch (p.build) {
         case 0:
           if (ws.bias) hipLaunchKernelGGL((gemm_w4p<FA, FB, 0, 1>), grid, block, 0, g.st, ws);
@@ -783,6 +888,7 @@
         MI_W4P_BUILDS_E4M3(MI_W4P)
         default: MI_NOT_COMPILED(p);
       }
+#undef MI_W4P192
 #undef MI_W4P
     }
     MI_CHECK_LAUNCH("mi_gemm (w4) launch");
diff --git a/llm_fp8_amd/pytorch/module.py b/llm_fp8_amd/pytorch/module.py
--- a/llm_fp8_amd/pytorch/module.py
+++ b/llm_fp8_amd/pytorch/module.py
@@ -562,7 +562,7 @@
 
 def _grouped_or_two(q, grad, w_col, x_col, dw_out, need_dgrad: bool, need_wgrad: bool):
     dgrad, wgrad, mx, fmt_b, fmt_f = q.operands(grad[0], w_col), q.operands(grad[1], x_col), q.mx, q.fmt_b, q.fmt_f
-    if need_dgrad and need_wgrad and ops.default_gemm_algo() in (0, 4, 47) and os.environ.get("LLM_FP8_AMD_NO_GROUPED_GEMM") != "1":
+    if need_dgrad and need_wgrad and ops.default_gemm_algo() in (0, 4, 39, 47) and os.environ.get("LLM_FP8_AMD_NO_GROUPED_GEMM") != "1":
         g8, wt8 = dgrad[0], dgrad[2 if mx else 1]
         M, N = g8.shape
         K = wt8.shape[0]
diff --git a/llm_fp8_amd/pytorch/ops.py b/llm_fp8_amd/pytorch/ops.py
--- a/llm_fp8_amd/pytorch/ops.py
+++ b/llm_fp8_amd/pytorch/ops.py
@@ -36,7 +36,7 @@
     d = torch.distributed
     if d.is_available() and d.is_initialized() and d.get_world_size() > 1:
         return 5
-    return 47 if os.environ.get("LLM_FP8_AMD_GEMM_W4", "1") != "0" else 0
+    return 39 if os.environ.get("LLM_FP8_AMD_GEMM_W4", "1") != "0" else 0
 
 
 def _stream() -> int:
@@ -219,7 +219,7 @@
 def _default_algo_for(M: int, N: int, K: int, out: Optional[torch.Tensor], out_dtype: torch.dtype, mx: bool) -> int:
     algo = default_gemm_algo()
     bf16 = out_dtype == torch.bfloat16 and (out is None or out.dtype == torch.bfloat16)
-    if ((mx and algo not in (0, 1, 4, 5)) or (algo == 3 and (M % 256 or N % 256 or K % 128)) or (algo == 47 and not bf16)
+    if ((mx and algo not in (0, 1, 4, 5)) or (algo == 3 and (M % 256 or N % 256 or K % 128)) or (algo in (39, 47) and not bf16)
             or (algo == 5 and ((M % 256 and M % 192) or (N % 256 and N % 192) or K % 256 or not bf16))):
         return 0
     return algo
```

Measured after the change: 89540 tokens/s (median of 4 runs). Within noise of the previous version (+0.9%).
